# Mistra-UEA/Mistra

Measured on AMD Instinct MI355X. Metric: chemistry-timesteps/sec (tot mechanism), higher is better.
Workload: dtype f64; 1 GPU; tot mechanism, 100000 synthetic cells per GPU (100000 total), INTEGRATE_t(0,10 s), Ros3 rtol 1e-3; perturbed captured BTZ96 cloud states; cells_per_gpu=100000, failed_cells=0, parallelism=cells sharded over 1 GPU(s), no data-path collective

## Files before the change

### __graft_entry__.py

```python
import os
import subprocess
import sys

REPO = os.path.dirname(os.path.abspath(__file__))
if REPO not in sys.path:
    sys.path.insert(0, REPO)


def build():
    from mistra_amd.build import build_lib
    lib = build_lib()
    assert os.path.exists(lib)
    subprocess.run(["make", "-s", "-C", os.path.join(REPO, "oracle")], check=True)
    subprocess.run(["make", "-s", "-C", os.path.join(REPO, "tests", "emu")], check=True)
    if os.path.isdir("/root/reference/src") and not os.path.exists(os.path.join(REPO, "oracle", "_ref", "libmistra_ref.so")):
        subprocess.run([os.path.join(REPO, "oracle", "build_ref.sh"), "lib"], check=True)
    if os.path.isdir("/root/reference/src") and not os.path.exists(os.path.join(REPO, "oracle", "_ref", "mistra_two_pass")):
        subprocess.run([os.path.join(REPO, "oracle", "build_ref.sh"), "model"], check=True)
        subprocess.run([os.path.join(REPO, "oracle", "build_two_pass.sh")], check=True)
    if os.path.isdir("/root/reference/src") and not os.path.exists(os.path.join(REPO, "oracle", "_ref", "mistra_drive")):
        subprocess.run([os.path.join(REPO, "oracle", "build_drive.sh")], check=True)
    gpu_model = os.path.join(REPO, "oracle", "_ref", "mistra_gpu")
    if os.path.isdir("/root/reference/src"):
        srcs = [os.path.join(REPO, "shim", f) for f in os.listdir(os.path.join(REPO, "shim")) if f.endswith(".f90")]
        srcs += [os.path.join(REPO, "oracle", f) for f in ("column_driver.f90", "two_pass_patch.py", "build_gpu_model.sh")]
        if not os.path.exists(gpu_model) or any(os.path.getmtime(f) > os.path.getmtime(gpu_model) for f in srcs):
            if os.path.getmtime(os.path.join(REPO, "oracle", "column_driver.f90")) > os.path.getmtime(os.path.join(REPO, "oracle", "_ref", "obj", "column_driver.o")):
                subprocess.run([os.path.join(REPO, "oracle", "build_ref.sh"), "model"], check=True)
            subprocess.run([os.path.join(REPO, "oracle", "build_gpu_model.sh")], check=True)
    import mistra_amd
    from mistra_amd import chem
    chem.lib()


def smoke():
    import numpy as np
    import torch
    from mistra_amd import chem
    from oracle.oracle import Oracle
    assert torch.cuda.is_available(), "smoke() needs a GPU"
    chem.init(0)
    for mech, n in (("tot", 8), ("gas", 4)):
        z = np.load(os.path.join(REPO, "tests", "golden", "integrate_%s.npz" % mech))
        var, fix, rconst = z["var_in"][:n], z["fix"][:n], z["rconst"][:n]
        dev = torch.device("cuda", 0)
        res = chem.integrate(mech, torch.tensor(var, device=dev), torch.tensor(fix, device=dev), torch.tensor(rconst, device=dev))
        torch.cuda.synchronize()
        got = res.var.cpu().numpy()
        want, ierr, st = Oracle(mech).integrate_batch(var, fix, rconst)
        assert np.all(res.ierr.cpu().numpy() == 1) and np.all(ierr == 1)
        floor = 1e-12 * np.abs(want).max(axis=1, keepdims=True)
        rel = np.abs(got - want) / (np.abs(want) + floor)
        assert rel.max() < 1e-6, "smoke parity failed for %s: %g" % (mech, rel.max())
        assert np.array_equal(res.stats.cpu().numpy()[:, 2], st[:, 2]), "step counts differ from the oracle"
        print("smoke %s: %d cells, max rel diff vs oracle %.3e, steps %s" % (mech, n, rel.max(), st[:, 2].tolist()))


if __name__ == "__main__":
    build()
    if "--smoke" in sys.argv:
        smoke()
```

### mistra_amd/csrc/capi.cpp

```cpp
#include "../../include/mistra_chem.h"

#include <dlfcn.h>
#include <hip/hip_runtime.h>

#include <algorithm>
#include <cstdio>
#include <cstdlib>
#include <cstring>
#include <mutex>
#include <string>
#include <thread>
#include <vector>

#include "kernel_args.hpp"
#include "mech_tables.hpp"
#include "pack.hpp"
#include "rates.hpp"
#include "ros3_kernel.hpp"
#include "schedule.hpp"

using namespace mistra;

namespace {

// ... 93 lines not shown
bool mistra::PackTable::load(const std::string& path, std::string* err) {
  FILE* f = std::fopen(path.c_str(), "rb");
  if (!f) { if (err) *err = "cannot open " + path; return false; }
  int32_t h[16];
  bool ok = std::fread(h, sizeof h, 1, f) == 1 && h[0] == 0x4B41504B && h[1] == 1;
  for (int i = 2; ok && i < 16; i++) ok = h[i] >= 0 && h[i] <= (1 << 20);
  ok = ok && h[2] > 0 && h[3] >= 0 && h[4] > 0 && h[5] > 0 && h[6] >= 1 && h[6] <= 8 && h[7] <= 1 && h[11] <= kBudSlots;
  auto rd = [&](std::vector<int32_t>& v, size_t n) { v.resize(n); return n == 0 || std::fread(v.data(), 4, n, f) == n; };
  if (ok) {
    nvar = h[2]; nfix = h[3]; j2 = h[4]; j6 = h[5]; nkc = h[6]; preclamp = h[7];
    ok = rd(pack, (size_t)h[8] * 4) && rd(fix, (size_t)h[9] * 3) && rd(unpack, (size_t)h[10] * 4) && rd(slot_id, (size_t)h[11]) &&
         rd(slot_first, (size_t)h[11] + 1) && rd(terms, (size_t)h[12] * 3) && rd(term_words, (size_t)h[13]) && rd(acc, (size_t)h[14] * 2) &&
         rd(envc, (size_t)h[15] * 2);
  }
  std::fclose(f);
  if (ok) {
    const int nspec = nvar + nfix, nl = j2 * nkc, ni = j6 * nkc, nterms = (int)terms.size() / 3, nwords = (int)term_words.size();
    for (int i = 0; ok && i < n_pack(); i++) {
      const int32_t* e = &pack[(size_t)4 * i];
      ok = e[0] >= 0 && e[0] < nspec && (e[1] == 0 || e[1] == 1) && e[2] >= 0 && e[2] < (e[1] == 0 ? nl : ni) && (e[3] == 0 || e[3] == 1);
    }
    for (int i = 0; ok && i < n_fix(); i++) {
      const int32_t* e = &fix[(size_t)3 * i];
      ok = e[0] >= 0 && e[0] < nspec && e[1] >= 0 && e[1] <= 3 && e[2] >= 0 && e[2] < 4;
    }
    for (int i = 0; ok && i < n_unpack(); i++) {
      const int32_t* e = &unpack[(size_t)4 * i];
      ok = (e[0] == 0 || e[0] == 1) && e[1] >= 0 && e[1] < (e[0] == 0 ? nl : ni) && e[2] >= 0 && e[2] < nvar && (e[3] == 0 || e[3] == 1);
    }
    for (int i = 0; ok && i < n_slots(); i++)
      ok = slot_id[(size_t)i] >= 1 && slot_id[(size_t)i] <= kBudSlots && slot_first[(size_t)i] >= 0 && slot_first[(size_t)i] <= slot_first[(size_t)i + 1] &&
           slot_first[(size_t)i + 1] <= nterms;
    for (int q = 0; ok && q < nterms; q++) {
      const int w0 = terms[(size_t)3 * q + 2], w1 = q + 1 < nterms ? terms[(size_t)3 * (q + 1) + 2] : nwords;
      ok = terms[(size_t)3 * q + 1] >= 0 && w0 >= 0 && w0 <= w1 && w1 <= nwords;
    }
    for (int32_t w : term_words) ok = ok && w >= 0 && w < nvar;
    for (size_t a = 0; ok && a < acc.size() / 2; a++) ok = acc[2 * a] >= 1 && acc[2 * a] <= acc[2 * a + 1] && acc[2 * a + 1] <= kBudSlots;
    for (int i = 0; ok && i < n_envc(); i++) ok = envc[(size_t)2 * i] >= 0 && envc[(size_t)2 * i + 1] >= 0 && envc[(size_t)2 * i + 1] < nspec;
  }
  if (!ok && err) *err = path + ": not a hand-over table";
  return ok;
}

bool mistra::KmtTable::load(const std::string& path, std::string* err) {
  FILE* f = std::fopen(path.c_str(), "r");
  if (!f) { if (err) *err = "cannot open " + path; return false; }
  bool ok = std::fscanf(f, "%d %d %d %d", &nx, &nka, &nkt, &nkc) == 4 && nx > 0 && nx <= 64;
  if (ok) {
    lex.resize((size_t)nx);
    for (int i = 0; ok && i < nx; i++) ok = std::fscanf(f, "%d", &lex[(size_t)i]) == 1;
  }
  std::fclose(f);
  if (!ok && err) *err = path + ": not a species list of fast_k_mt";
  return ok;
}

bool mistra::LiqTable::load(const std::string& path, std::string* err) {
  FILE* f = std::fopen(path.c_str(), "rb");
  if (!f) { if (err) *err = "cannot open " + path; return false; }
  int32_t h[8];
  double d[3];
  bool ok = std::fread(h, sizeof h, 1, f) == 1 && h[0] == 0x5451494C && h[1] == 1 && h[2] > 0 && h[2] <= 4096 && h[3] >= 0 && h[3] <= h[2] &&
            h[4] >= 0 && h[4] <= h[2] && h[5] >= 1 && h[5] <= 8 && h[6] >= 0 && h[6] <= 1 << 20 && std::fread(d, sizeof d, 1, f) == 1;
  std::vector<int32_t> hj, hk, ej;
  std::vector<double> a0, b0;
  auto rdi = [&](std::vector<int32_t>& v, size_t n) { v.resize(n); return n == 0 || std::fread(v.data(), 4, n, f) == n; };
  auto rdd = [&](std::vector<double>& v, size_t n) { v.resize(n); return n == 0 || std::fread(v.data(), 8, n, f) == n; };
  if (ok) {
    nspec = h[2]; nh = h[3]; ne = h[4]; nkc_eq = h[5]; nfac = h[6];
    henry_tref = d[0]; henry_fct = d[1]; equil_tref = d[2];
    ok = rdi(hj, (size_t)nh) && rdi(hk, (size_t)nh) && rdd(a0, (size_t)nh) && rdd(b0, (size_t)nh) && rdi(ej, (size_t)ne) && rdi(foff, (size_t)ne + 1) &&
         rdi(boff, (size_t)ne + 1) && rdi(fkind, (size_t)nfac) && rdi(farg, (size_t)nfac) && rdd(fa, (size_t)nfac) && rdd(fb, (size_t)nfac);
  }
  std::fclose(f);
  if (ok) {
    h_kind.assign((size_t)nspec, -1); h_a0.assign((size_t)nspec, 0.0); h_b0.assign((size_t)nspec, 0.0); e_of.assign((size_t)nspec, -1);
    for (int i = 0; ok && i < nh; i++) {
      ok = hj[(size_t)i] >= 1 && hj[(size_t)i] <= nspec && (hk[(size_t)i] == 0 || hk[(size_t)i] == 1);
      if (ok) { const size_t j = (size_t)hj[(size_t)i] - 1; h_kind[j] = hk[(size_t)i]; h_a0[j] = a0[(size_t)i]; h_b0[j] = b0[(size_t)i]; }
    }
    for (int i = 0; ok && i < ne; i++) {
      ok = ej[(size_t)i] >= 1 && ej[(size_t)i] <= nspec && foff[(size_t)i] >= 0 && foff[(size_t)i] < boff[(size_t)i] && boff[(size_t)i] < foff[(size_t)i + 1] &&
           foff[(size_t)i + 1] <= nfac;
      if (ok) e_of[(size_t)ej[(size_t)i] - 1] = i;
    }
    for (int i = 0; ok && i < nfac; i++) ok = fkind[(size_t)i] >= 0 && fkind[(size_t)i] <= 3 && (fkind[(size_t)i] != 3 || (farg[(size_t)i] >= 1 && farg[(size_t)i] <= 4096));
  }
  if (!ok && err) *err = path + ": not a table of Henry / equilibrium constants";
  return ok;
}

bool mistra::VmeanTable::load(const std::string& path, std::string* err) {
  FILE* f = std::fopen(path.c_str(), "rb");
  if (!f) { if (err) *err = "cannot open " + path; return false; }
  int32_t h[8];
  bool ok = std::fread(h, sizeof h, 1, f) == 1 && h[0] == 0x544E4D56 && h[1] == 1 && h[2] > 0 && h[2] <= 4096 && h[3] >= 0 && h[3] <= h[2] &&
            std::fread(&coef, sizeof coef, 1, f) == 1 && coef > 0.0;
  std::vector<int32_t> j;
  std::vector<double> m;
  if (ok) {
    nspec = h[2];
    j.resize((size_t)h[3]); m.resize((size_t)h[3]);
    ok = (h[3] == 0 || std::fread(j.data(), 4, j.size(), f) == j.size()) && (h[3] == 0 || std::fread(m.data(), 8, m.size(), f) == m.size());
  }
  std::fclose(f);
  if (ok) {
    mass.assign((size_t)nspec, 0.0);
    for (size_t i = 0; ok && i < j.size(); i++) {
      ok = j[i] >= 1 && j[i] <= nspec && m[i] > 0.0;
      if (ok) mass[(size_t)j[i] - 1] = m[i];
    }
  }
  if (!ok && err) *err = path + ": not a table of molar masses of v_mean";
  return ok;
}

namespace {

struct VmBufs {
  DevBuf<uint32_t> wave_base, recs;
  DevBuf<uint16_t> blk_n;
  int nrounds = 0;
  hipError_t upload(const VmProgram& P) {
    nrounds = P.nbarriers;
    hipError_t e;
    if ((e = wave_base.upload(P.wave_base)) != hipSuccess) return e;
    if ((e = blk_n.upload(P.blk_n)) != hipSuccess) return e;
    return recs.upload(P.recs);
  }
  VmDev dev() const { return VmDev{wave_base.p, blk_n.p, recs.p, nrounds}; }
  void release() { wave_base.release(); recs.release(); blk_n.release(); }
};

struct GsBufs {
  DevBuf<uint32_t> wave_base, recs;
  DevBuf<uint16_t> rows;
  hipError_t upload(const GsumProgram& P) {
    hipError_t e;
    if ((e = wave_base.upload(P.wave_base)) != hipSuccess) return e;
    if ((e = rows.upload(P.rows)) != hipSuccess) return e;
    return recs.upload(P.recs);
  }
  GsDev dev() const { return GsDev{wave_base.p, rows.p, recs.p}; }
  void release() { wave_base.release(); recs.release(); rows.release(); }
};


struct KernelBufs {
  int n_temps = 0, lu_scale_slots = 0;
  DevBuf<double> consts;
  DevBuf<uint64_t> fun_fac, jac_fac;
  DevBuf<uint16_t> jvs_pos, zero_pos, diag_pos, schur_cells;
  GsBufs vdot, jvs;
  VmBufs lu, solve_head_fwd, solve_head_bwd;
  DevBuf<uint32_t> tail_fwd, tail_bwd, tail_fwd_addr[2], tail_bwd_addr[2], lu_scale, dense_rows;
  int upload(const MechTables& t, const KernelSchedule& K) {
    n_temps = K.n_temps;
    lu_scale_slots = K.lu_scale.nslots;
    HIP_TRY(consts.upload(t.consts));
    HIP_TRY(fun_fac.upload(K.fun_fac));
    HIP_TRY(jac_fac.upload(K.jac_fac));
    HIP_TRY(jvs_pos.upload(K.jvs_pos));
    HIP_TRY(zero_pos.upload(K.zero_pos));
    HIP_TRY(diag_pos.upload(K.diag_pos));
    HIP_TRY(vdot.upload(K.vdot));
    HIP_TRY(jvs.upload(K.jvs));
    HIP_TRY(lu.upload(K.lu));
    HIP_TRY(solve_head_fwd.upload(K.solve_head_fwd));
    HIP_TRY(solve_head_bwd.upload(K.solve_head_bwd));
    HIP_TRY(tail_fwd.upload(K.tail.fwd));
    HIP_TRY(tail_bwd.upload(K.tail.bwd));
    for (int r = 0; r < 2; r++) {
      HIP_TRY(tail_fwd_addr[r].upload(K.tail.fwd_addr[r]));
      HIP_TRY(tail_bwd_addr[r].upload(K.tail.bwd_addr[r]));
    }
    HIP_TRY(lu_scale.upload(K.lu_scale.recs));
    HIP_TRY(dense_rows.upload(K.dense.row_info));
    HIP_TRY(schur_cells.upload(K.dense.schur_cells));
    return 0;
  }
  void release() {
    consts.release(); fun_fac.release(); jac_fac.release(); jvs_pos.release(); zero_pos.release(); diag_pos.release(); schur_cells.release();
    vdot.release(); jvs.release(); lu.release(); solve_head_fwd.release(); solve_head_bwd.release();
    tail_fwd.release(); tail_bwd.release(); lu_scale.release(); dense_rows.release();
    for (int r = 0; r < 2; r++) { tail_fwd_addr[r].release(); tail_bwd_addr[r].release(); }
  }
};

struct RatesBufs {
  bool ready = false;
  int nreact = 0, nenv = 0;
  DevBuf<double> consts;
  DevBuf<int32_t> offs, words, fslot;
  int upload(const RatesTable& T) {
    HIP_TRY(consts.upload(T.consts));
    HIP_TRY(offs.upload(T.offs));
    HIP_TRY(words.upload(T.words));
    HIP_TRY(fslot.upload(T.fslot));
    nreact = T.nreact; nenv = T.nenv;
    ready = true;
    return 0;
  }
  RatesDev dev() const { return RatesDev{consts.p, offs.p, words.p, fslot.p, nreact, nenv}; }
  void release() { consts.release(); offs.release(); words.release(); fslot.release(); ready = false; }
};

struct PackBufs {
  bool ready = false, maps_ready = false;
  PackTable tab;
  DevBuf<int32_t> pack, fix, unpack, slot_id, slot_first, terms, words, acc, envc, a_ptr, a_fac;
  DevBuf<int32_t> gas_m2k, gas_k2m, rad_m2k, rad_k2m;
  int j1 = 0, j5 = 0;
  int upload(const MechTables& t) {
    HIP_TRY(pack.upload(tab.pack)); HIP_TRY(fix.upload(tab.fix)); HIP_TRY(unpack.upload(tab.unpack));
    HIP_TRY(slot_id.upload(tab.slot_id)); HIP_TRY(slot_first.upload(tab.slot_first)); HIP_TRY(terms.upload(tab.terms));
    HIP_TRY(words.upload(tab.term_words)); HIP_TRY(acc.upload(tab.acc)); HIP_TRY(envc.upload(tab.envc));
    HIP_TRY(a_ptr.upload(t.a_ptr)); HIP_TRY(a_fac.upload(t.a_fac));
    ready = true;
    return 0;
  }
  int set_maps(int n1, const int32_t* g_m2k, const int32_t* g_k2m, int n5, const int32_t* r_m2k, const int32_t* r_k2m) {
    HIP_TRY(gas_m2k.upload(std::vector<int32_t>(g_m2k, g_m2k + 2 * (size_t)n1)));
    HIP_TRY(gas_k2m.upload(std::vector<int32_t>(g_k2m, g_k2m + (size_t)n1)));
    HIP_TRY(rad_m2k.upload(std::vector<int32_t>(r_m2k, r_m2k + 2 * (size_t)n5)));
    HIP_TRY(rad_k2m.upload(std::vector<int32_t>(r_k2m, r_k2m + (size_t)n5)));
    j1 = n1; j5 = n5;
    maps_ready = true;
    return 0;
  }
  PackDev dev(int nreact, const double* consts) const {
    const PackTable& T = tab;
    return PackDev{pack.p, fix.p, unpack.p, slot_id.p, slot_first.p, terms.p, words.p, acc.p, envc.p,
                   T.n_pack(), T.n_fix(), T.n_unpack(), T.n_slots(), (int)T.terms.size() / 3, (int)T.term_words.size(), (int)T.acc.size() / 2, T.n_envc(),
                   T.nvar, T.nfix, nreact, T.j2, T.j6, T.nkc, T.preclamp, gas_m2k.p, gas_k2m.p, rad_m2k.p, rad_k2m.p, j1, j5, a_ptr.p, a_fac.p, consts};
  }
  void release() {
    pack.release(); fix.release(); unpack.release(); slot_id.release(); slot_first.release(); terms.release(); words.release(); acc.release();
    envc.release(); a_ptr.release(); a_fac.release(); gas_m2k.release(); gas_k2m.release(); rad_m2k.release(); rad_k2m.release();
    ready = maps_ready = false;
  }
};

struct KmtBufs {
  bool ready = false;
  KmtTable tab;
  DevBuf<int32_t> lex;
  int upload() {
    HIP_TRY(lex.upload(tab.lex));
    ready = true;
    return 0;
  }
  KmtDev dev(int nspec, int ka, int ifeed, int nkc_l) const { return KmtDev{lex.p, {0}, tab.nx, tab.nka, tab.nkt, tab.nkc, nspec, ka, ifeed, nkc_l}; }
  void release() { lex.release(); ready = false; }
};

struct LiqBufs {
  bool ready = false;
  LiqTable tab;
  DevBuf<int32_t> h_kind, e_of, foff, boff, fkind, farg;
  DevBuf<double> h_a0, h_b0, fa, fb;
  int upload() {
    HIP_TRY(h_kind.upload(tab.h_kind)); HIP_TRY(e_of.upload(tab.e_of)); HIP_TRY(foff.upload(tab.foff)); HIP_TRY(boff.upload(tab.boff));
    HIP_TRY(fkind.upload(tab.fkind)); HIP_TRY(farg.upload(tab.farg)); HIP_TRY(h_a0.upload(tab.h_a0)); HIP_TRY(h_b0.upload(tab.h_b0));
    HIP_TRY(fa.upload(tab.fa)); HIP_TRY(fb.upload(tab.fb));
    ready = true;
    return 0;
  }
  LiqDev dev() const {
    return LiqDev{h_kind.p, e_of.p, foff.p, boff.p, fkind.p, farg.p, h_a0.p, h_b0.p, fa.p, fb.p, tab.nspec, tab.nkc_eq, tab.henry_tref, tab.henry_fct, tab.equil_tref};
  }
  void release() {
    h_kind.release(); e_of.release(); foff.release(); boff.release(); fkind.release(); farg.release(); h_a0.release(); h_b0.release();
    fa.release(); fb.release(); ready = false;
  }
};

struct StcBufs {
  bool ready = false;
  StcoeffTable tab;
  DevBuf<double> consts[4];
  DevBuf<int32_t> offs[4], words[4];
  int upload() {
    for (int i = 0; i < 4; i++) {
      HIP_TRY(consts[i].upload(tab.v[i].consts)); HIP_TRY(offs[i].upload(tab.v[i].offs)); HIP_TRY(words[i].upload(tab.v[i].words));
    }
    ready = true;
    return 0;
  }
  RatesDev dev(int v) const { return RatesDev{consts[v].p, offs[v].p, words[v].p, nullptr, tab.v[v].nreact, tab.v[v].nenv}; }
  void release() {
    for (int i = 0; i < 4; i++) { consts[i].release(); offs[i].release(); words[i].release(); }
    ready = false;
  }
};

struct VmeanBufs {
  bool ready = false;
  VmeanTable tab;
  DevBuf<double> mass;
  int upload() {
    HIP_TRY(mass.upload(tab.mass));
    ready = true;
    return 0;
  }
  void release() { mass.release(); ready = false; }
};

enum : unsigned { kNeedRates = 1, kNeedPackTable = 2, kNeedMaps = 4, kNeedPack = kNeedPackTable | kNeedMaps, kNeedKmt = 8, kNeedLiq = 16, kNeedStc = 32, kNeedVmean = 64 };


struct Staging {
  char *dev = nullptr, *host = nullptr;
  size_t cap = 0;
  hipStream_t st = nullptr;
  hipError_t ensure(size_t bytes) {
    if (!st)
      if (hipError_t e = hipStreamCreateWithFlags(&st, hipStreamNonBlocking)) return e;
    if (bytes <= cap) return hipSuccess;
    free_blocks();
    const size_t want = bytes + bytes / 2;
    if (hipError_t e = hipMalloc(reinterpret_cast<void**>(&dev), want)) return e;
    if (hipError_t e = hipHostMalloc(reinterpret_cast<void**>(&host), want, hipHostMallocDefault)) return e;
    cap = want;
    return hipSuccess;
  }
  template <class T = double>
  T* d(size_t off) const { return reinterpret_cast<T*>(dev + off); }
  template <class T = double>
  T* h(size_t off) const { return reinterpret_cast<T*>(host + off); }
  void free_blocks() {
    if (dev) (void)hipFree(dev);
    if (host) (void)hipHostFree(host);
    dev = host = nullptr; cap = 0;
  }
  void release() {
    free_blocks();
    if (st) (void)hipStreamDestroy(st);
    st = nullptr;
  }
};

struct Layout {
  size_t end = 0;
  size_t take(size_t bytes) {
    const size_t at = end;
    end += (bytes + 255) & ~(size_t)255;
    return at;
  }
};

struct DriveLayout {
  size_t nl = 0, j1 = 0, j5 = 0, nsl = 0, nsi = 0, nv = 0, nf = 0, nr = 0, ne = 0;
  size_t s1 = 0, s3 = 0, sl1 = 0, si = 0, bg = 0, bgs = 0, io_end = 0, scal = 0, env = 0, in_end = 0;
  size_t th = 0, hl = 0, ierr = 0, stats = 0, cp = 0, out_end = 0, var = 0, fix = 0, rct = 0, end = 0;
};

struct MechState {
  bool ready = false;
  int nt = 0;
  MechTables tab;
  std::string text;
  KernelBufs k;
  RatesBufs rates;
  PackBufs pack;
  KmtBufs kmt;
  LiqBufs liq;
  StcBufs stc;
  VmeanBufs vmean;
  DevBuf<double> d_rct;
  DevBuf<double> s_var, s_fix, s_rct, s_th, s_env;
  DevBuf<int32_t> s_ierr, s_stats, s_sing;
  size_t sing_start = 0, sing_count = 0;
  bool sing_one = false;
  int32_t one_sing[8] = {0, 0, 0, 0, 0, 0, 0, 0};
  Staging drive;
  Staging one;
  struct PendingDrive {
    bool active = false;
    DriveLayout lay;
    std::vector<int32_t> layer, level;
    double *s1 = nullptr, *s3 = nullptr, *sl1 = nullptr, *sion1 = nullptr, *bg = nullptr, *bgs = nullptr, *t_h = nullptr, *c_packed = nullptr;
    int32_t *ierr = nullptr, *stats = nullptr;
    int nrxn = 0;
  } pend;
  void release() {
    k.release(); rates.release(); pack.release(); kmt.release(); liq.release(); stc.release(); vmean.release();
    d_rct.release();
    s_var.release(); s_fix.release(); s_rct.release(); s_th.release(); s_env.release(); s_ierr.release(); s_stats.release(); s_sing.release();
    sing_count = 0; sing_one = false;
    drive.release(); one.release();
    pend = PendingDrive{};
    ready = false;
  }
};

struct DeviceState {
  int id = -1;
  MechState mech[3];
  bool lds_configured[3] = {false, false, false};
  void release() {
    if (id >= 0) (void)hipSetDevice(id);
    for (auto& m : mech) m.release();
    for (bool& c : lds_configured) c = false;
    id = -1;
  }
};

std::mutex g_mu;
bool g_inited = false;
int g_max_steps = 100000;
std::vector<DeviceState> g_devs;

Staging g_liq;
struct PinnedRanges {
  std::vector<std::pair<const char*, size_t>> r;
  bool contains(const void* p, size_t n) const {
    const char* c = static_cast<const char*>(p);
    for (const auto& x : r)
      if (c >= x.first && c + n <= x.first + x.second) return true;
    return false;
  }
  void release() {
    for (const auto& x : r) (void)hipHostUnregister(const_cast<char*>(x.first));
    r.clear();
  }
} g_pinned;

void release_all() {
  if (!g_devs.empty() && g_devs[0].id >= 0) (void)hipSetDevice(g_devs[0].id);
  g_pinned.release();
  g_liq.release();
  for (auto& d : g_devs) d.release();
  g_devs.clear();
  g_inited = false;
}

std::string mech_dir() {
  if (const char* e = std::getenv("MISTRA_MECH_DIR")) return e;
  Dl_info info;
  if (dladdr(reinterpret_cast<const void*>(&mistra_chem_init), &info) && info.dli_fname) {
    std::string p = info.dli_fname;
    size_t k = p.rfind('/');
    std::string dir = k == std::string::npos ? "." : p.substr(0, k);
    return dir + "/../mech";
  }
  return "mech";
}

int default_nt(int mech) { return mech == MISTRA_MECH_GAS ? kGasNT : mech == MISTRA_MECH_AER ? kAerNT : kTotNT; }

template <class MT>
bool traits_match(const MechTables& t, int n_jnz, int tail_regs, bool scale_pass, const DenseTail& dense) {
  return dense.nd == MT::DENSE_ND && dense.kb == MT::DENSE_KB && tail_regs == MT::TAIL_REGS && scale_pass == MT::SCALE_PASS && t.nvar == MT::NVAR && t.nfix == MT::NFIX && t.nreact == MT::NREACT && t.nnz == MT::NNZ && t.nb == MT::NB &&
         t.nconst == MT::NCONST && n_jnz == MT::NJNZ;
}

int setup_mech(DeviceState& D, int mech) {
  MechState& S = D.mech[mech];
  const std::string name = kMechName[mech], base = mech_dir() + "/" + name;
  std::string err;
  if (!S.tab.load(base + ".mech", &err)) return fail(err);
  S.nt = default_nt(mech);
  const bool nt_ok = (mech == MISTRA_MECH_GAS && S.nt == kGasNT) || (mech == MISTRA_MECH_AER && S.nt == kAerNT) ||
                     (mech == MISTRA_MECH_TOT && S.nt == kTotNT);
  if (!nt_ok) return fail(std::string("no kernel instantiated for workgroup size ") + std::to_string(S.nt) + " of " + kMechName[mech]);
  const uint32_t ab_base = 8u * (uint32_t)(mech == MISTRA_MECH_GAS   ? LdsLayout<GasTraits, kGasNT>::AB
                                           : mech == MISTRA_MECH_AER ? LdsLayout<AerTraits, kAerNT>::AB
                                                                     : LdsLayout<TotTraits, kTotNT>::AB);
  KernelSchedule K;
  try {
    const int max_temps = mech == MISTRA_MECH_GAS ? GasTraits::MAX_TEMPS : mech == MISTRA_MECH_AER ? AerTraits::MAX_TEMPS : TotTraits::MAX_TEMPS;
    const DenseConfig dc = dense_config(S.tab);
    const uint32_t jb_base = 8u * (uint32_t)(mech == MISTRA_MECH_GAS   ? LdsLayout<GasTraits, kGasNT>::JB
                                             : mech == MISTRA_MECH_AER ? LdsLayout<AerTraits, kAerNT>::JB
                                                                       : LdsLayout<TotTraits, kTotNT>::JB);
    K = build_kernel_schedule(S.tab, S.nt, ab_base, max_temps, dc.nd, dc.kb, jb_base);
  } catch (const std::exception& ex) {
    return fail(std::string("schedule compiler: ") + ex.what());
  }
  bool ok = mech == MISTRA_MECH_GAS   ? traits_match<GasTraits>(S.tab, K.n_jnz, K.tail.regs, K.lu_scale.nslots > 0, K.dense)
            : mech == MISTRA_MECH_AER ? traits_match<AerTraits>(S.tab, K.n_jnz, K.tail.regs, K.lu_scale.nslots > 0, K.dense)
                                      : traits_match<TotTraits>(S.tab, K.n_jnz, K.tail.regs, K.lu_scale.nslots > 0, K.dense);
  if (!ok) return fail(name + ": mechanism table does not match the compiled kernel sizes");
  S.text = name + ": " + describe(K);
  if (int rc = S.k.upload(S.tab, K)) return rc;
  const int nspec = S.tab.nvar + S.tab.nfix;
  RatesTable R;
  if (R.load(base + ".rates", &err)) {
    if (R.nreact != S.tab.nreact) return fail(name + ".rates does not belong to this mechanism");
    if (int rc = S.rates.upload(R)) return rc;
  }
  if (S.pack.tab.load(base + ".pack", &err)) {
    const PackTable& T = S.pack.tab;
    if (T.nvar != S.tab.nvar || T.nfix != S.tab.nfix) return fail(name + ".pack does not belong to this mechanism");
    for (size_t q = 0; q < T.terms.size() / 3; q++)
      if (T.terms[3 * q + 1] >= S.tab.nreact) return fail(name + ".pack: a budget term names a reaction the mechanism does not have");
    for (int i = 0; i < T.n_envc(); i++)
      if (S.rates.ready && T.envc[(size_t)2 * i] >= S.rates.nenv) return fail(name + ".pack: a concentration slot lies outside the rate evaluator's input");
    if (int rc = S.pack.upload(S.tab)) return rc;
  }
  if (S.kmt.tab.load(base + ".kmt", &err)) {
    for (int32_t i : S.kmt.tab.lex)
      if (i < 1 || i > nspec) return fail(name + ".kmt does not belong to this mechanism");
    if (int rc = S.kmt.upload()) return rc;
  }
  if (S.liq.tab.load(base + ".liq", &err)) {
    if (S.liq.tab.nspec != nspec) return fail(name + ".liq does not belong to this mechanism");
    if (int rc = S.liq.upload()) return rc;
  }
  if (S.stc.tab.load(base + ".stcoeff", &err)) {
    if (S.stc.tab.v[0].nreact != nspec) return fail(name + ".stcoeff does not belong to this mechanism");
    if (int rc = S.stc.upload()) return rc;
  }
  if (S.vmean.tab.load(base + ".vmean", &err)) {
    if (S.vmean.tab.nspec != nspec) return fail(name + ".vmean does not belong to this mechanism");
    if (int rc = S.vmean.upload()) return rc;
  }
  S.ready = true;
  return 0;
}

int launch(DeviceState& D, int mech, const KernelArgs& a, hipStream_t stream) {
  hipError_t e = hipErrorInvalidValue;
  if (mech == MISTRA_MECH_GAS) e = launch_ros3<GasTraits, kGasNT>(a, stream, &D.lds_configured[mech]);
  else if (mech == MISTRA_MECH_AER) e = launch_ros3<AerTraits, kAerNT>(a, stream, &D.lds_configured[mech]);
  else e = launch_ros3<TotTraits, kTotNT>(a, stream, &D.lds_configured[mech]);
  if (e != hipSuccess) return fail(std::string("kernel launch: ") + hipGetErrorString(e));
  return 0;
}

KernelArgs make_args(const MechState& S, int ncell, const double* var_in, const double* fix, const double* rconst, double tin,
                     double tout, double* var_out, int32_t* ierr, int32_t* stats, double* th) {
  const KernelBufs& k = S.k;
  KernelArgs a;
  a.var_in = var_in; a.fix = fix; a.rconst = rconst; a.var_out = var_out; a.ierr = ierr; a.stats = stats;
  a.texit_hexit = th; a.h_last = nullptr; a.hstart = nullptr; a.prof = nullptr; a.dump = nullptr; a.sing_rows = nullptr; a.n_temps = k.n_temps; a.max_steps = g_max_steps; a.tin = tin; a.tout = tout; a.ncell = ncell;
  a.consts = k.consts.p; a.fun_fac = k.fun_fac.p; a.jac_fac = k.jac_fac.p; a.jvs_pos = k.jvs_pos.p;
  a.zero_pos = k.zero_pos.p; a.diag_pos = k.diag_pos.p;
  a.vdot = k.vdot.dev(); a.jvs = k.jvs.dev(); a.lu = k.lu.dev();
#ifdef MISTRA_DIAG_ENV
  if (const char* cut = std::getenv("MISTRA_DIAG_LU_ROUNDS"))
    a.lu.nrounds = std::max(1, std::min(a.lu.nrounds, std::atoi(cut)));
#endif
  a.solve_head_fwd = k.solve_head_fwd.dev(); a.solve_head_bwd = k.solve_head_bwd.dev();
  a.tail = TailDev{k.tail_fwd.p, k.tail_bwd.p, {k.tail_fwd_addr[0].p, k.tail_fwd_addr[1].p}, {k.tail_bwd_addr[0].p, k.tail_bwd_addr[1].p}};
  a.lu_scale = ScaleDev{k.lu_scale.p, k.lu_scale_slots, k.lu_scale_slots + VM_LOOKAHEAD_ROWS};
  a.dense = DenseDev{k.dense_rows.p, k.schur_cells.p};
  return a;
}

PackDev pack_dev(const MechState& S) { return S.pack.dev(S.tab.nreact, S.k.consts.p); }

int check_call(int mech, int ncell) {
  if (mech < 0 || mech > 2) return fail("unknown mechanism id");
  if (ncell < 0) return fail("negative cell count");
  if (!g_inited || g_devs.empty() || !g_devs[0].mech[mech].ready) return fail("mistra_chem_init has not been called (or failed)");
  return 0;
}

int require(const MechState& S, int mech, unsigned need) {
  const std::string m = kMechName[mech];
  if ((need & kNeedPackTable) && !S.pack.ready) return fail("no hand-over table for the " + m + " mechanism");
  if ((need & kNeedMaps) && !S.pack.maps_ready) return fail("mistra_chem_set_species_maps has not been called for the " + m + " mechanism");
  if ((need & kNeedRates) && !S.rates.ready) return fail("no device rate table for the " + m + " mechanism");
  if ((need & kNeedKmt) && !S.kmt.ready) return fail("the " + m + " mechanism has no mass-transfer routine (fast_k_mt_a: aer, fast_k_mt_t: tot)");
  if ((need & kNeedLiq) && !S.liq.ready)
    return fail("the " + m + " mechanism has no liquid-phase routines (henry_a / equil_co_a: aer, henry_t / equil_co_t: tot)");
  if ((need & kNeedStc) && !S.stc.ready) return fail("the " + m + " mechanism has no st_coeff routine (st_coeff_a: aer, st_coeff_t: tot)");
  if ((need & kNeedVmean) && !S.vmean.ready) return fail("the " + m + " mechanism has no v_mean routine (v_mean_a: aer, v_mean_t: tot)");
  return 0;
}

struct Slot {
  DeviceState* D = nullptr;
  MechState* S = nullptr;
};

int on_device(int mech, int ncell, const void* p, const char* what, unsigned need, Slot* t) {
  if (int rc = check_call(mech, ncell)) return rc;
  hipPointerAttribute_t attr;
  if (hipPointerGetAttributes(&attr, p) != hipSuccess) return fail(std::string(what) + " is not a device pointer");
  DeviceState* D = nullptr;
  for (auto& d : g_devs)
    if (d.id == attr.device) { D = &d; break; }
  if (!D) return fail("the buffers live on device " + std::to_string(attr.device) + ", which mistra_chem_init(_devices) did not set up");
  if (int rc = require(D->mech[mech], mech, need)) return rc;
  HIP_TRY(hipSetDevice(D->id));
  *t = Slot{D, &D->mech[mech]};
  return 0;
}

int on_primary(int mech, unsigned need, bool mutates, Slot* t) {
  DeviceState& D = g_devs[0];
  MechState& S = D.mech[mech];
  if (mutates && S.pend.active)
    return fail(std::string("a column step of the ") + kMechName[mech] + " mechanism is open (mistra_chem_drive_begin): fetch it with mistra_chem_drive_end first");
  if (int rc = require(S, mech, need)) return rc;
  HIP_TRY(hipSetDevice(D.id));
  *t = Slot{&D, &S};
  return 0;
}

int init_locked(int n, const int* ids) {
  int count = 0;
  hipError_t e = hipGetDeviceCount(&count);
  if (e != hipSuccess || count <= 0) return fail("no HIP device available (this library has no CPU path)");
  if (n <= 0 || n > 64) return fail("device count out of range");
  std::vector<int> want((size_t)n);
  for (int i = 0; i < n; i++) {
    want[(size_t)i] = ids ? ids[i] : i;
    if (want[(size_t)i] < 0 || want[(size_t)i] >= count) return fail("device index out of range");
  }
  bool same = g_inited && g_devs.size() == want.size();
  for (size_t i = 0; same && i < want.size(); i++) same = g_devs[i].id == want[i];
  if (same) {
    HIP_TRY(hipSetDevice(g_devs[0].id));
    return 0;
  }
  release_all();
  g_devs.resize(want.size());
  for (size_t i = 0; i < want.size(); i++) {
    HIP_TRY(hipSetDevice(want[i]));
    g_devs[i].id = want[i];
    for (int mech = 0; mech < 3; mech++)
      if (int rc = setup_mech(g_devs[i], mech)) return rc;
  }
  HIP_TRY(hipSetDevice(g_devs[0].id));
  g_inited = true;
  return 0;
}

int integrate_host_on(DeviceState& D, int mech, int ncell, const double* var_in, const double* fix, const double* rconst, double tin,
                      double tout, double* var_out, int32_t* ierr, int32_t* stats, double* t_h, size_t batch_start = 0,
                      const double* env = nullptr) {
  HIP_TRY(hipSetDevice(D.id));
  MechState& S = D.mech[mech];
  const size_t nv = (size_t)kDims[mech].nvar, nf = (size_t)kDims[mech].nfix, nr = (size_t)kDims[mech].nreact, nc = (size_t)ncell;
  HIP_TRY(S.s_var.reserve(nc * nv));
  HIP_TRY(S.s_fix.reserve(nc * nf));
  HIP_TRY(S.s_rct.reserve(nc * nr));
  HIP_TRY(S.s_ierr.reserve(nc));
  HIP_TRY(S.s_stats.reserve(nc * 8));
  HIP_TRY(S.s_sing.reserve(nc * 8));
  if (t_h) HIP_TRY(S.s_th.reserve(nc * 3));
  HIP_TRY(hipMemcpy(S.s_var.p, var_in, nc * nv * sizeof(double), hipMemcpyHostToDevice));
  HIP_TRY(hipMemcpy(S.s_fix.p, fix, nc * nf * sizeof(double), hipMemcpyHostToDevice));
  if (env) {
    const size_t ne = (size_t)S.rates.nenv;
    HIP_TRY(S.s_env.reserve(nc * ne));
    HIP_TRY(hipMemcpy(S.s_env.p, env, nc * ne * sizeof(double), hipMemcpyHostToDevice));
    LAUNCH_TRY(launch_update_rconst(S.rates.dev(), S.s_env.p, S.s_rct.p, ncell, nullptr));
  } else {
    HIP_TRY(hipMemcpy(S.s_rct.p, rconst, nc * nr * sizeof(double), hipMemcpyHostToDevice));
  }
  KernelArgs a = make_args(S, ncell, S.s_var.p, S.s_fix.p, S.s_rct.p, tin, tout, S.s_var.p, S.s_ierr.p, S.s_stats.p, t_h ? S.s_th.p : nullptr);
  if (t_h) a.h_last = S.s_th.p + 2 * nc;
  a.sing_rows = S.s_sing.p;
  S.sing_start = batch_start; S.sing_count = nc; S.sing_one = false;
  DevBuf<unsigned long long> prof;
#ifdef MISTRA_DIAG_ENV
  const bool profile = std::getenv("MISTRA_CHEM_PROFILE") != nullptr;
#else
  const bool profile = false;
#endif
  if (profile) {
    HIP_TRY(prof.reserve(nc * kProfSlots));
    a.prof = prof.p;
  }
  if (int rc = launch(D, mech, a, nullptr)) return rc;
  HIP_TRY(hipDeviceSynchronize());
  if (profile) {
    std::vector<unsigned long long> h(nc * kProfSlots);
    HIP_TRY(hipMemcpy(h.data(), prof.p, nc * kProfSlots * sizeof(unsigned long long), hipMemcpyDeviceToHost));
    double sum[kProfSlots] = {0};
    for (size_t c = 0; c < nc; c++)
      for (int k = 0; k < kProfSlots; k++) sum[k] += (double)h[c * kProfSlots + k];
    const char* names[kProfSlots] = {"fun", "jac", "prepare", "lu", "solve(rest)", "norm", "other", "total", "solve_head_fwd", "solve_tail", "solve_head_bwd", "lu_scale", "lu_dense", "jac_products", "jac_sums", "fun_products"};
    std::fprintf(stderr, "[mistra_chem profile] %s, %zu cells, mean shader-clock ticks per cell:", kMechName[mech], nc);
    for (int k = 0; k < kProfSlots; k++) std::fprintf(stderr, " %s=%.0f (%.1f%%)", names[k], sum[k] / nc, 100.0 * sum[k] / sum[7]);
    std::fprintf(stderr, "\n");
    prof.release();
  }
  HIP_TRY(hipMemcpy(var_out, S.s_var.p, nc * nv * sizeof(double), hipMemcpyDeviceToHost));
  if (ierr) HIP_TRY(hipMemcpy(ierr, S.s_ierr.p, nc * sizeof(int32_t), hipMemcpyDeviceToHost));
  if (stats) HIP_TRY(hipMemcpy(stats, S.s_stats.p, nc * 8 * sizeof(int32_t), hipMemcpyDeviceToHost));
  if (t_h) {
    std::vector<double> h(nc * 3);
    HIP_TRY(hipMemcpy(h.data(), S.s_th.p, nc * 3 * sizeof(double), hipMemcpyDeviceToHost));
    for (size_t c = 0; c < nc; c++) { t_h[3 * c] = h[2 * c]; t_h[3 * c + 1] = h[2 * c + 1]; t_h[3 * c + 2] = h[2 * nc + c]; }
  }
  return 0;
}
// ... 871 lines not shown
```

### mistra_amd/csrc/kernel_args.hpp

```cpp
#pragma once
#include <cstdint>

namespace mistra {

constexpr int kProfSlots = 16;
constexpr int kVmSweepUpdPerRec = 3;

struct VmDev {
  const uint32_t* wave_base;
  const uint16_t* blk_n;
  const uint32_t* recs;
  int nrounds;
};

struct GsDev {
  const uint32_t* wave_base;
  const uint16_t* rows;
  const uint32_t* recs;
};

struct ScaleDev {
  const uint32_t* recs;
  int nslots;
  int wave_slots;
};

struct TailDev {
  const uint32_t* fwd;
  const uint32_t* bwd;
  const uint32_t* fwd_addr[2];
  const uint32_t* bwd_addr[2];
};

struct DenseDev {
  const uint32_t* row_info;
  const uint16_t* schur_cells;
};

struct KernelArgs {
  const double* var_in;
  const double* fix;
  const double* rconst;
  double* var_out;
  int32_t* ierr;
  int32_t* stats;
  double* texit_hexit;
  const double* hstart;
  double* h_last;
  int32_t* sing_rows;
  double* dump;
  unsigned long long* prof;
  double tin, tout;
  int32_t ncell;
  int32_t n_temps;
  int32_t max_steps;
  const double* consts;
  const uint64_t* fun_fac;
  const uint64_t* jac_fac;
  const uint16_t* jvs_pos;
  const uint16_t* zero_pos;
  const uint16_t* diag_pos;
  GsDev vdot, jvs;
  VmDev lu, solve_head_fwd, solve_head_bwd;
  ScaleDev lu_scale;
  TailDev tail;
  DenseDev dense;
};

}
```

### mistra_amd/csrc/ros3_kernel.hip

```cpp
#include <hip/hip_runtime.h>

#include <cstdint>
#include <type_traits>

#include "kernel_args.hpp"
#include "ros3_kernel.hpp"

namespace mistra {

namespace {

constexpr uint16_t kPosDiag = 0x8000, kPosNone = 0xFFFF;
constexpr int kRingSlots = 8;

typedef uint32_t u32x4 __attribute__((ext_vector_type(4)));
typedef float f32x4 __attribute__((ext_vector_type(4)));

template <class T>
using gptr = const T __attribute__((address_space(1)))*;
template <class T>
using gptr_mut = T __attribute__((address_space(1)))*;
template <class T>
__device__ __forceinline__ gptr<T> G_(const T* p) { return (gptr<T>)p; }
template <class T>
__device__ __forceinline__ gptr_mut<T> GM_(T* p) { return (gptr_mut<T>)p; }

typedef __attribute__((address_space(3))) double lds_f64;
__device__ __forceinline__ uint32_t lds_addr(const void* p) {
  return (uint32_t)(uintptr_t)(__attribute__((address_space(3))) const void*)p;
}
__device__ __forceinline__ double lds_ld(uint32_t addr) { return *(const lds_f64*)(uintptr_t)addr; }
__device__ __forceinline__ void lds_st(uint32_t addr, double v) { *(lds_f64*)(uintptr_t)addr = v; }

__device__ __forceinline__ void lds_barrier() {
  __builtin_amdgcn_fence(__ATOMIC_RELEASE, "workgroup", "local");
  __builtin_amdgcn_s_barrier();
  __builtin_amdgcn_fence(__ATOMIC_ACQUIRE, "workgroup", "local");
}

constexpr double kRosA1 = 1.0;
constexpr double kRosC1 = -0.10156171083877702091975600115545e+01;
constexpr double kRosC2 = 0.40759956452537699824805835358067e+01;
constexpr double kRosC3 = 0.92076794298330791242156818474003e+01;
constexpr double kRosM1 = 0.1e+01;
constexpr double kRosM2 = 0.61697947043828245592553615689730e+01;
constexpr double kRosM3 = -0.42772256543218573326238373806514e+00;
constexpr double kRosE1 = 0.5e+00;
constexpr double kRosE2 = -0.29079558716805469821718236208017e+01;
constexpr double kRosE3 = 0.22354069897811569627360909276199e+00;
constexpr double kRosGamma1 = 0.43586652150845899941601945119356e+00;
[[maybe_unused]] constexpr double kRosGamma2 = 0.24291996454816804366592249683314e+00;
[[maybe_unused]] constexpr double kRosGamma3 = 0.21851380027664058511513169485832e+01;
constexpr double kRosElo = 3.0;

__device__ __attribute__((noinline)) double err_root(double err) { return pow(err, 1.0 / kRosElo); }

__device__ __forceinline__ double wave_uniform(double v) {
  const uint64_t u = __builtin_bit_cast(uint64_t, v);
  const uint32_t lo = (uint32_t)__builtin_amdgcn_readfirstlane((int)(uint32_t)u), hi = (uint32_t)__builtin_amdgcn_readfirstlane((int)(uint32_t)(u >> 32));
  return __builtin_bit_cast(double, (uint64_t)lo | ((uint64_t)hi << 32));
}

__device__ __forceinline__ double scalar_const(double v) {
  const uint64_t u = __builtin_bit_cast(uint64_t, v);
  uint32_t lo = (uint32_t)u, hi = (uint32_t)(u >> 32);
  asm volatile("" : "+s"(lo), "+s"(hi));
  return __builtin_bit_cast(double, (uint64_t)lo | ((uint64_t)hi << 32));
}

template <int CTRL>
__device__ __forceinline__ double dpp_partner(double v) {
  const uint64_t u = __builtin_bit_cast(uint64_t, v);
  const int lo = __builtin_amdgcn_update_dpp(0, (int)(uint32_t)u, CTRL, 0xf, 0xf, false);
  const int hi = __builtin_amdgcn_update_dpp(0, (int)(uint32_t)(u >> 32), CTRL, 0xf, 0xf, false);
  return __builtin_bit_cast(double, (uint64_t)(uint32_t)lo | ((uint64_t)(uint32_t)hi << 32));
}
__device__ __forceinline__ double wave_sum(double v) {
  v += dpp_partner<0xB1>(v);
  v += dpp_partner<0x4E>(v);
  v += dpp_partner<0x141>(v);
  v += dpp_partner<0x140>(v);
  {
    const uint64_t u = __builtin_bit_cast(uint64_t, v);
    const auto l = __builtin_amdgcn_permlane16_swap((uint32_t)u, (uint32_t)u, false, false);
    const auto h = __builtin_amdgcn_permlane16_swap((uint32_t)(u >> 32), (uint32_t)(u >> 32), false, false);
    v = __builtin_bit_cast(double, (uint64_t)l[0] | ((uint64_t)h[0] << 32)) + __builtin_bit_cast(double, (uint64_t)l[1] | ((uint64_t)h[1] << 32));
  }
  {
    const uint64_t u = __builtin_bit_cast(uint64_t, v);
    const auto l = __builtin_amdgcn_permlane32_swap((uint32_t)u, (uint32_t)u, false, false);
    const auto h = __builtin_amdgcn_permlane32_swap((uint32_t)(u >> 32), (uint32_t)(u >> 32), false, false);
    v = __builtin_bit_cast(double, (uint64_t)l[0] | ((uint64_t)h[0] << 32)) + __builtin_bit_cast(double, (uint64_t)l[1] | ((uint64_t)h[1] << 32));
  }
  return v;
}

__device__ __forceinline__ double fmin_f(double a, double b) { return (a < b || b != b) ? a : b; }
__device__ __forceinline__ double fmax_f(double a, double b) { return (a > b || b != b) ? a : b; }

template <bool LOW, int K, int BYTE_OFFSET = 0>
__device__ __forceinline__ void vm_ring_load(gptr<u32x4> p) {
#define MISTRA_RING_LOAD(R0, R1, R2, R3)                                                                              \
  asm volatile("global_load_dwordx4 v[" #R0 ":" #R3 "], %0, off offset:%1" : : "v"(p), "n"(BYTE_OFFSET)             \
               : "memory", "v" #R0, "v" #R1, "v" #R2, "v" #R3)
  if constexpr (LOW) {
    if constexpr (K == 0) MISTRA_RING_LOAD(64, 65, 66, 67);
    else if constexpr (K == 1) MISTRA_RING_LOAD(68, 69, 70, 71);
    else if constexpr (K == 2) MISTRA_RING_LOAD(80, 81, 82, 83);
    else if constexpr (K == 3) MISTRA_RING_LOAD(84, 85, 86, 87);
    else if constexpr (K == 4) MISTRA_RING_LOAD(96, 97, 98, 99);
    else if constexpr (K == 5) MISTRA_RING_LOAD(100, 101, 102, 103);
    else if constexpr (K == 6) MISTRA_RING_LOAD(112, 113, 114, 115);
    else MISTRA_RING_LOAD(116, 117, 118, 119);
  } else {
    if constexpr (K == 0) MISTRA_RING_LOAD(192, 193, 194, 195);
    else if constexpr (K == 1) MISTRA_RING_LOAD(196, 197, 198, 199);
    else if constexpr (K == 2) MISTRA_RING_LOAD(208, 209, 210, 211);
    else if constexpr (K == 3) MISTRA_RING_LOAD(212, 213, 214, 215);
    else if constexpr (K == 4) MISTRA_RING_LOAD(224, 225, 226, 227);
    else if constexpr (K == 5) MISTRA_RING_LOAD(228, 229, 230, 231);
    else if constexpr (K == 6) MISTRA_RING_LOAD(240, 241, 242, 243);
    else MISTRA_RING_LOAD(244, 245, 246, 247);
  }
#undef MISTRA_RING_LOAD
}

struct RingBase { uint64_t b0, b1; };
__device__ __forceinline__ RingBase ring_base(const void* p) {
  const uint64_t u = (uint64_t)(uintptr_t)p;
  uint32_t lo, hi;
  asm volatile("v_readfirstlane_b32 %0, %2\n\tv_readfirstlane_b32 %1, %3\n\ts_nop 4" : "=s"(lo), "=s"(hi) : "v"((uint32_t)u), "v"((uint32_t)(u >> 32)));
  const uint64_t b = (uint64_t)lo | ((uint64_t)hi << 32);
  return RingBase{b, b + 4096};
}
__device__ __forceinline__ void ring_advance(RingBase& r, uint32_t bytes) { r.b0 += bytes; r.b1 += bytes; }
template <bool LOW, int K, int ROW>
__device__ __forceinline__ void vm_ring_load_s(const RingBase& r, uint32_t voff) {
  static_assert(ROW >= 0 && ROW <= 7, "row within the two 4-KiB windows");
#define MISTRA_RING_LOAD_S(R0, R1, R2, R3)                                                                                    \
  asm volatile("global_load_dwordx4 v[" #R0 ":" #R3 "], %0, %1 offset:%2" : : "v"(voff), "s"(ROW < 4 ? r.b0 : r.b1), "n"((ROW % 4) * 1024) \
               : "memory", "v" #R0, "v" #R1, "v" #R2, "v" #R3)
  if constexpr (LOW) {
    if constexpr (K == 0) MISTRA_RING_LOAD_S(64, 65, 66, 67);
    else if constexpr (K == 1) MISTRA_RING_LOAD_S(68, 69, 70, 71);
    else if constexpr (K == 2) MISTRA_RING_LOAD_S(80, 81, 82, 83);
    else if constexpr (K == 3) MISTRA_RING_LOAD_S(84, 85, 86, 87);
    else if constexpr (K == 4) MISTRA_RING_LOAD_S(96, 97, 98, 99);
    else if constexpr (K == 5) MISTRA_RING_LOAD_S(100, 101, 102, 103);
    else if constexpr (K == 6) MISTRA_RING_LOAD_S(112, 113, 114, 115);
    else MISTRA_RING_LOAD_S(116, 117, 118, 119);
  } else {
    if constexpr (K == 0) MISTRA_RING_LOAD_S(192, 193, 194, 195);
    else if constexpr (K == 1) MISTRA_RING_LOAD_S(196, 197, 198, 199);
    else if constexpr (K == 2) MISTRA_RING_LOAD_S(208, 209, 210, 211);
    else if constexpr (K == 3) MISTRA_RING_LOAD_S(212, 213, 214, 215);
    else if constexpr (K == 4) MISTRA_RING_LOAD_S(224, 225, 226, 227);
    else if constexpr (K == 5) MISTRA_RING_LOAD_S(228, 229, 230, 231);
    else if constexpr (K == 6) MISTRA_RING_LOAD_S(240, 241, 242, 243);
    else MISTRA_RING_LOAD_S(244, 245, 246, 247);
  }
#undef MISTRA_RING_LOAD_S
}

template <bool LOW, int K, int IMM>
__device__ __forceinline__ void vm_ring_load_at(uint64_t sbase, uint32_t voff) {
  static_assert(IMM >= 0 && IMM < 4096, "13-bit signed immediate offset");
#define MISTRA_RING_LOAD_AT(R0, R1, R2, R3)                                                                                   \
  asm volatile("global_load_dwordx4 v[" #R0 ":" #R3 "], %0, %1 offset:%2" : : "v"(voff), "s"(sbase), "n"(IMM)                \
               : "memory", "v" #R0, "v" #R1, "v" #R2, "v" #R3)
// ... 396 lines not shown
    } else {
      base = tb[0] + (uint64_t)(TS::NB + G - TS::NG) * 4096u;
    }
    vm_ring_load_at<LOW, K0, 0>(base, voff); vm_ring_load_at<LOW, K0 + 1, 1024>(base, voff);
    vm_ring_load_at<LOW, K0 + 2, 2048>(base, voff); vm_ring_load_at<LOW, K0 + 3, 3072>(base, voff);
  };
  asm volatile("s_waitcnt vmcnt(0)" : : : "memory");
  load(std::integral_constant<int, 0>());
  load(std::integral_constant<int, 1>());
  double c[16];
  {
    double g[16];
    tail_gather<LOW, 0>(g);
    load(std::integral_constant<int, 2>());
#pragma unroll
    for (int j = 0; j < 16; j++) c[j] = g[TS::bw(0) ? 15 - j : j];
  }
#define MISTRA_TAIL_STEP(S)                                                                                               \
  if constexpr ((S) < TS::NS) {                                                                                          \
    if constexpr ((S) == TS::NF) {                                                                                       \
      _Pragma("unroll") for (int r = 0; r < R; r++) x[r] = x[r] * rd[r];                                                 \
    }                                                                                                                    \
    tail_block<TS, (S), LOW>(x, c, load);                                                                                \
  }
  MISTRA_TAIL_STEP(0) MISTRA_TAIL_STEP(1) MISTRA_TAIL_STEP(2) MISTRA_TAIL_STEP(3) MISTRA_TAIL_STEP(4) MISTRA_TAIL_STEP(5) MISTRA_TAIL_STEP(6) MISTRA_TAIL_STEP(7)
  MISTRA_TAIL_STEP(8) MISTRA_TAIL_STEP(9) MISTRA_TAIL_STEP(10) MISTRA_TAIL_STEP(11) MISTRA_TAIL_STEP(12) MISTRA_TAIL_STEP(13) MISTRA_TAIL_STEP(14) MISTRA_TAIL_STEP(15)
#undef MISTRA_TAIL_STEP
  asm volatile("s_waitcnt vmcnt(0)" : : : "memory");
#pragma unroll
  for (int r = 0; r < R; r++) lds_st(xb + 8 * (r * 64 + lane), x[r]);
}

__device__ __forceinline__ double readlane_f64(double v, int l) {
  const uint64_t u = __builtin_bit_cast(uint64_t, v);
  const uint32_t lo = (uint32_t)__builtin_amdgcn_readlane((int)(uint32_t)u, l);
  const uint32_t hi = (uint32_t)__builtin_amdgcn_readlane((int)(uint32_t)(u >> 32), l);
  return __builtin_bit_cast(double, (uint64_t)lo | ((uint64_t)hi << 32));
}

template <int R, int FWD_FROM, bool LOW>
__device__ __attribute__((noinline)) void tail_solve_columns(const TailDev T, uint32_t xb, uint32_t rb, int lane) {
  constexpr int FWD_END = R;
  constexpr bool FORWARD = FWD_FROM < FWD_END;
  constexpr uint32_t mb = 0;
  double x[R], rd[R];
  const uint32_t voff = 16u * (uint32_t)lane;
  static_assert(R == 1 || R == 2, "one or two 64-row registers");
  uint32_t three = 3;
  asm volatile("" : "+v"(three));
#pragma unroll
  for (int r = 0; r < R; r++) x[r] = lds_ld(xb + 8 * (r * 64 + lane));
#define MISTRA_TAIL_OPERANDS(BUF, K, PENDING)                                           \
  {                                                                                     \
    uint32_t alo[4], ahi[4];                                                            \
    vm_ring_take_cells<LOW, K, PENDING, true, R == 2>(alo, ahi, three);                 \
    _Pragma("unroll") for (int c = 0; c < 4; c++) {                                     \
      BUF[c][0] = lds_ld(mb + alo[c]);                                                  \
      if constexpr (R == 2) BUF[c][1] = lds_ld(mb + ahi[c]);                            \
    }                                                                                   \
  }
#define MISTRA_TAIL_PIN _Pragma("unroll") for (int r = 0; r < R; r++) asm volatile("" : "+v"(x[r]));
  double opa[4][R], opb[4][R];
  if constexpr (FORWARD) {
    RingBase tp = ring_base(T.fwd + FWD_FROM * 16 * 64 * 4);
    asm volatile("s_waitcnt vmcnt(0)" : : : "memory");
    vm_ring_load_s<LOW, 0, 0>(tp, voff); vm_ring_load_s<LOW, 1, 1>(tp, voff); vm_ring_load_s<LOW, 2, 2>(tp, voff); vm_ring_load_s<LOW, 3, 3>(tp, voff);
    vm_ring_load_s<LOW, 4, 4>(tp, voff); vm_ring_load_s<LOW, 5, 5>(tp, voff); vm_ring_load_s<LOW, 6, 6>(tp, voff); vm_ring_load_s<LOW, 7, 7>(tp, voff);
    ring_advance(tp, kRingSlots * 1024);
    MISTRA_TAIL_OPERANDS(opa, 0, 7)
    vm_ring_load_s<LOW, 0, 0>(tp, voff);
#pragma unroll
    for (int rq = FWD_FROM; rq < FWD_END; rq++) {
      for (int gb = 0; gb < 16; gb += kRingSlots) {
#define MISTRA_TAIL_FWD(K, CUR, NXT)                                                    \
        {                                                                               \
          MISTRA_TAIL_OPERANDS(NXT, (K + 1) % kRingSlots, 7)                                 \
          if constexpr (K + 1 == kRingSlots) ring_advance(tp, kRingSlots * 1024);            \
          vm_ring_load_s<LOW, (K + 1) % kRingSlots, (K + 1) % kRingSlots>(tp, voff);         \
          _Pragma("unroll") for (int c = 0; c < 4; c++) {                               \
            const double xq = readlane_f64(x[rq], 4 * (gb + K) + c);                    \
            _Pragma("unroll") for (int r = rq; r < R; r++) x[r] = __builtin_fma(-CUR[c][r], xq, x[r]); \
          }                                                                             \
          MISTRA_TAIL_PIN                                                               \
        }
        MISTRA_TAIL_FWD(0, opa, opb) MISTRA_TAIL_FWD(1, opb, opa) MISTRA_TAIL_FWD(2, opa, opb) MISTRA_TAIL_FWD(3, opb, opa)
        MISTRA_TAIL_FWD(4, opa, opb) MISTRA_TAIL_FWD(5, opb, opa) MISTRA_TAIL_FWD(6, opa, opb) MISTRA_TAIL_FWD(7, opb, opa)
#undef MISTRA_TAIL_FWD
      }
    }
  }
  {
    RingBase tp = ring_base(T.bwd);
    asm volatile("s_waitcnt vmcnt(0)" : : : "memory");
    vm_ring_load_s<LOW, 0, 0>(tp, voff); vm_ring_load_s<LOW, 1, 1>(tp, voff); vm_ring_load_s<LOW, 2, 2>(tp, voff); vm_ring_load_s<LOW, 3, 3>(tp, voff);
    vm_ring_load_s<LOW, 4, 4>(tp, voff); vm_ring_load_s<LOW, 5, 5>(tp, voff); vm_ring_load_s<LOW, 6, 6>(tp, voff); vm_ring_load_s<LOW, 7, 7>(tp, voff);
    ring_advance(tp, kRingSlots * 1024);
#pragma unroll
    for (int r = 0; r < R; r++) rd[r] = lds_ld(rb + 8 * (r * 64 + lane));
#pragma unroll
    for (int r = 0; r < R; r++) x[r] = x[r] * rd[r];
    MISTRA_TAIL_OPERANDS(opa, 0, 7)
    vm_ring_load_s<LOW, 0, 0>(tp, voff);
#pragma unroll
    for (int rq = R - 1; rq >= 0; rq--) {
      for (int gb = 0; gb < 16; gb += kRingSlots) {
#define MISTRA_TAIL_BWD(K, CUR, NXT)                                                    \
        {                                                                               \
          MISTRA_TAIL_OPERANDS(NXT, (K + 1) % kRingSlots, 7)                                 \
          if constexpr (K + 1 == kRingSlots) ring_advance(tp, kRingSlots * 1024);            \
          vm_ring_load_s<LOW, (K + 1) % kRingSlots, (K + 1) % kRingSlots>(tp, voff);         \
          _Pragma("unroll") for (int c = 0; c < 4; c++) {                               \
            const double xq = readlane_f64(x[rq], 63 - (4 * (gb + K) + c));             \
            _Pragma("unroll") for (int r = 0; r <= rq; r++) x[r] = __builtin_fma(-CUR[c][r], xq, x[r]); \
          }                                                                             \
          MISTRA_TAIL_PIN                                                               \
        }
        MISTRA_TAIL_BWD(0, opa, opb) MISTRA_TAIL_BWD(1, opb, opa) MISTRA_TAIL_BWD(2, opa, opb) MISTRA_TAIL_BWD(3, opb, opa)
        MISTRA_TAIL_BWD(4, opa, opb) MISTRA_TAIL_BWD(5, opb, opa) MISTRA_TAIL_BWD(6, opa, opb) MISTRA_TAIL_BWD(7, opb, opa)
#undef MISTRA_TAIL_BWD
      }
    }
  }
#undef MISTRA_TAIL_OPERANDS
#undef MISTRA_TAIL_PIN
  asm volatile("s_waitcnt vmcnt(0)" : : : "memory");
#pragma unroll
  for (int r = 0; r < R; r++) lds_st(xb + 8 * (r * 64 + lane), x[r]);
}

#include "gsum_exec_asm.inc"
template <int NT, bool LOW>
__device__ __attribute__((noinline)) void gsum_run(const GsDev P, uint32_t row0, int rows, int lane, uint32_t out_addr, uint32_t out_stride) {
  int n = __builtin_amdgcn_readfirstlane(rows);
  const uint64_t recs = reinterpret_cast<uint64_t>(P.recs) + (uint64_t)(uint32_t)__builtin_amdgcn_readfirstlane((int)row0) * 2048u;
  const uint64_t b0 = (uint64_t)(uint32_t)__builtin_amdgcn_readfirstlane((int)(uint32_t)recs) |
                      ((uint64_t)(uint32_t)__builtin_amdgcn_readfirstlane((int)(uint32_t)(recs >> 32)) << 32);
  const uint64_t b1 = b0 + 4096u;
  uint32_t voff = (uint32_t)lane * 32u;
  double acc = -0.0;
  const double mzero = -0.0;
  double xA0, xA1, xA2, xA3, xB0, xB1, xB2, xB3, cA0, cA1, cA2, cA3, cB0, cB1, cB2, cB3;
  uint32_t ad, flA, flB;
#define MISTRA_GSUM_OPERANDS                                                                                                                   \
  [acc] "+&v"(acc), [ad] "=&v"(ad), [xA0] "=&v"(xA0), [xA1] "=&v"(xA1), [xA2] "=&v"(xA2), [xA3] "=&v"(xA3), [xB0] "=&v"(xB0), [xB1] "=&v"(xB1),    \
      [xB2] "=&v"(xB2), [xB3] "=&v"(xB3), [cA0] "=&v"(cA0), [cA1] "=&v"(cA1), [cA2] "=&v"(cA2), [cA3] "=&v"(cA3), [cB0] "=&v"(cB0),               \
      [cB1] "=&v"(cB1), [cB2] "=&v"(cB2), [cB3] "=&v"(cB3), [flA] "=&s"(flA), [flB] "=&s"(flB), [n] "+s"(n), [voff] "+&v"(voff),               \
      [out] "+&v"(out_addr)                                                                                                                    \
      : [b0] "s"(b0), [b1] "s"(b1), [stride] "v"(out_stride), [mzero] "v"(mzero)
  if constexpr (LOW) asm volatile(MISTRA_GSUM_ASM_LOW : MISTRA_GSUM_OPERANDS : "memory", "scc", MISTRA_GSUM_CLOBBER_LOW);
  else asm volatile(MISTRA_GSUM_ASM_HIGH : MISTRA_GSUM_OPERANDS : "memory", "scc", MISTRA_GSUM_CLOBBER_HIGH);
#undef MISTRA_GSUM_OPERANDS
}

template <int NT, bool LOW>
__device__ __attribute__((noinline)) void scale_run(const ScaleDev P, int wave, int lane) {
  const int n = __builtin_amdgcn_readfirstlane(P.nslots);
  gptr<u32x4> rp = G_(reinterpret_cast<const u32x4*>(P.recs)) + ((size_t)wave * (size_t)P.wave_slots * 64 + lane);
  asm volatile("s_waitcnt vmcnt(0)" : : : "memory");
  vm_ring_load<LOW, 0>(rp);       vm_ring_load<LOW, 1>(rp + 64);  vm_ring_load<LOW, 2>(rp + 128); vm_ring_load<LOW, 3>(rp + 192);
  vm_ring_load<LOW, 4>(rp + 256); vm_ring_load<LOW, 5>(rp + 320); vm_ring_load<LOW, 6>(rp + 384); vm_ring_load<LOW, 7>(rp + 448);
  rp += kRingSlots * 64;
  for (int i = 0; i < n; i += kRingSlots) {
#define MISTRA_SCALE_GROUP(K)                                                        \
    {                                                                                \
      const u32x4 a0 = vm_ring_take<LOW, K>();     vm_ring_load<LOW, K>(rp + K * 64);         \
      const u32x4 a1 = vm_ring_take<LOW, K + 1>(); vm_ring_load<LOW, K + 1>(rp + (K + 1) * 64); \
      const u32x4 a2 = vm_ring_take<LOW, K + 2>(); vm_ring_load<LOW, K + 2>(rp + (K + 2) * 64); \
      const u32x4 a3 = vm_ring_take<LOW, K + 3>(); vm_ring_load<LOW, K + 3>(rp + (K + 3) * 64); \
      const double v0 = lds_ld(a0.x), f0 = lds_ld(a0.y), v1 = lds_ld(a0.z), f1 = lds_ld(a0.w); \
      const double v2 = lds_ld(a1.x), f2 = lds_ld(a1.y), v3 = lds_ld(a1.z), f3 = lds_ld(a1.w); \
      const double v4 = lds_ld(a2.x), f4 = lds_ld(a2.y), v5 = lds_ld(a2.z), f5 = lds_ld(a2.w); \
      const double v6 = lds_ld(a3.x), f6 = lds_ld(a3.y), v7 = lds_ld(a3.z), f7 = lds_ld(a3.w); \
      lds_st(a0.x, v0 * f0); lds_st(a0.z, v1 * f1); lds_st(a1.x, v2 * f2); lds_st(a1.z, v3 * f3); \
      lds_st(a2.x, v4 * f4); lds_st(a2.z, v5 * f5); lds_st(a3.x, v6 * f6); lds_st(a3.z, v7 * f7); \
    }
    MISTRA_SCALE_GROUP(0) MISTRA_SCALE_GROUP(4)
#undef MISTRA_SCALE_GROUP
    rp += kRingSlots * 64;
  }
  asm volatile("s_waitcnt vmcnt(0)" : : : "memory");
}

#ifdef MISTRA_DIAG_STAMPS
__device__ unsigned long long g_dense_stamps[16];
#define MISTRA_STAMP(var) const unsigned long long var = clock64();
#define MISTRA_STAMP_ADD(slot, expr) if (threadIdx.x == 0) atomicAdd(&g_dense_stamps[slot], (unsigned long long)(expr));
#else
#define MISTRA_STAMP(var)
#define MISTRA_STAMP_ADD(slot, expr)
#endif
typedef double f64x4 __attribute__((ext_vector_type(4)));
typedef uint32_t u32x2 __attribute__((ext_vector_type(2)));
typedef __attribute__((address_space(3))) f64x4 lds_f64x4;
__device__ __forceinline__ f64x4 lds_ld4(uint32_t addr) { return *(const lds_f64x4*)(uintptr_t)addr; }
__device__ __forceinline__ void lds_st4(uint32_t addr, f64x4 v) { *(lds_f64x4*)(uintptr_t)addr = v; }

__device__ __forceinline__ uint32_t dense_slot(const u32x4 info, const uint32_t c, const uint32_t zero) {
  const uint64_t absent = (uint64_t)info.y | ((uint64_t)info.z << 32);
  const uint32_t idx = info.x + c - (uint32_t)__builtin_popcountll(absent & ((1ull << c) - 1ull));
  return ((absent >> c) & 1ull) ? zero : 8u * idx;
}
typedef __attribute__((address_space(3))) u32x4 lds_u32x4;
__device__ __forceinline__ u32x4 lds_ldu4(uint32_t addr) { return *(const lds_u32x4*)(uintptr_t)addr; }

__device__ __forceinline__ bool dense_is_storer(const int wave) { return wave == 1 || wave == 2 || wave == 3 || wave == 5; }
template <class MT, int NT>
__device__ __forceinline__ void dense_store_panel(const int P, const int wave, const int lane) {
  constexpr uint32_t NNZ = MT::NNZ, NVAR = MT::NVAR, H = NVAR - 64, ZERO = 8u * (NNZ + NVAR);
  constexpr uint32_t PB = 8u * (uint32_t)LdsLayout<MT, NT>::PANEL, BC = PB + 8192u, INFO = 8u * (uint32_t)LdsLayout<MT, NT>::DINFO;
  const uint32_t PL = PB + (uint32_t)(P & 1) * 4096u, PU = PL + 2048u;
  const int J0P = 4 * P, khalf = (wave == 3 || wave == 5) ? 2 : 0;
  const f64x4 rcp = lds_ld4(BC + 1024u + 32u * (uint32_t)(P & 1));
  if (wave & 1) {
    if (wave != 5) {
      const f64x4 a = lds_ld4(PL + 32u * lane);
      const u32x4 mine = lds_ldu4(INFO + 16u * lane);
      const double a0 = khalf ? a[2] : a[0], a1 = khalf ? a[3] : a[1];
      const uint32_t at0 = dense_slot(mine, (uint32_t)(J0P + khalf), ZERO), at1 = dense_slot(mine, (uint32_t)(J0P + khalf + 1), ZERO);
      if (lane > J0P + khalf && at0 != ZERO) lds_st(at0, a0);
      if (lane > J0P + khalf + 1 && at1 != ZERO) lds_st(at1, a1);
      if (wave == 1 && lane >= J0P && lane < J0P + 4) {
        const int k = lane - J0P;
        lds_st(8u * (NNZ + NVAR + 4u + H + (uint32_t)lane), k == 0 ? rcp[0] : k == 1 ? rcp[1] : k == 2 ? rcp[2] : rcp[3]);
      }
      return;
    }
  }
  {
    const f64x4 b = lds_ld4(PU + 32u * lane);
    const double b0 = khalf ? b[2] : b[0], b1 = khalf ? b[3] : b[1], r0 = khalf ? rcp[2] : rcp[0], r1 = khalf ? rcp[3] : rcp[1];
    const uint32_t at0 = dense_slot(lds_ldu4(INFO + 16u * (uint32_t)(J0P + khalf)), (uint32_t)lane, ZERO);
    const uint32_t at1 = dense_slot(lds_ldu4(INFO + 16u * (uint32_t)(J0P + khalf + 1)), (uint32_t)lane, ZERO);
    if (lane >= J0P + khalf && at0 != ZERO) lds_st(at0, lane == J0P + khalf ? b0 : b0 * r0);
    if (lane >= J0P + khalf + 1 && at1 != ZERO) lds_st(at1, lane == J0P + khalf + 1 ? b1 : b1 * r1);
  }
}

template <class MT, int NT>
__device__ __forceinline__ void dense_panel(f64x4& T0, f64x4& T1, const int P, const int wave, const int lane
#ifdef MISTRA_DIAG_STAMPS
                                            , unsigned long long (&acc)[5]
#endif
) {
  const int K = P >> 2, S = P & 3, J0P = 4 * P, K2 = (J0P + 4) >> 4;
  constexpr uint32_t PB = 8u * (uint32_t)LdsLayout<MT, NT>::PANEL, BC = PB + 8192u;
  const uint32_t PL = PB + (uint32_t)(P & 1) * 4096u, PU = PL + 2048u;
  const int I = wave >> 1, J0 = 2 * (wave & 1);
  const uint32_t lrow = (uint32_t)(lane >> 4), lcol = (uint32_t)(lane & 15);
  MISTRA_STAMP(ta)
  if (I >= K && (wave & 1) == (K >> 1)) {
    const bool odd = K & 1;
    const double t0 = odd ? T1[0] : T0[0], t1 = odd ? T1[1] : T0[1], t2 = odd ? T1[2] : T0[2], t3 = odd ? T1[3] : T0[3];
    if ((int)(lcol >> 2) == S) {
      const uint32_t at = PL + 8u * ((16u * I + lrow) * 4u + (lcol & 3u));
      lds_st(at, t0); lds_st(at + 128u, t1); lds_st(at + 256u, t2); lds_st(at + 384u, t3);
    }
  }
  if (I == K) {
    if (J0 >= K) lds_st(PU + 8u * ((16u * J0 + lcol) * 4u + lrow), S == 0 ? T0[0] : S == 1 ? T0[1] : S == 2 ? T0[2] : T0[3]);
    if (J0 + 1 >= K) lds_st(PU + 8u * ((16u * (J0 + 1) + lcol) * 4u + lrow), S == 0 ? T1[0] : S == 1 ? T1[1] : S == 2 ? T1[2] : T1[3]);
  }
  lds_barrier();
  MISTRA_STAMP(tb)
  if (wave == 0) {
    f64x4 a = lds_ld4(PL + 32u * lane), b = lds_ld4(PU + 32u * lane);
    const f64x4 c0 = lds_ld4(PU + 32u * (uint32_t)J0P), c1 = lds_ld4(PU + 32u * (uint32_t)(J0P + 1));
    const f64x4 c2 = lds_ld4(PU + 32u * (uint32_t)(J0P + 2)), c3 = lds_ld4(PU + 32u * (uint32_t)(J0P + 3));
    f64x4 rcp;
    rcp[0] = 1.0 / c0[0];
    const double l10 = c0[1] * rcp[0], l20 = c0[2] * rcp[0], l30 = c0[3] * rcp[0];
    const double u01 = c1[0], u02 = c2[0], u03 = c3[0];
    const double d11 = __builtin_fma(-l10, u01, c1[1]), d12 = __builtin_fma(-l10, u02, c2[1]), d13 = __builtin_fma(-l10, u03, c3[1]);
    double d21 = __builtin_fma(-l20, u01, c1[2]), d22 = __builtin_fma(-l20, u02, c2[2]), d23 = __builtin_fma(-l20, u03, c3[2]);
    double d31 = __builtin_fma(-l30, u01, c1[3]), d32 = __builtin_fma(-l30, u02, c2[3]), d33 = __builtin_fma(-l30, u03, c3[3]);
    rcp[1] = 1.0 / d11;
    const double l21 = d21 * rcp[1], l31 = d31 * rcp[1];
    d22 = __builtin_fma(-l21, d12, d22); d23 = __builtin_fma(-l21, d13, d23);
    d32 = __builtin_fma(-l31, d12, d32); d33 = __builtin_fma(-l31, d13, d33);
    rcp[2] = 1.0 / d22;
    const double l32 = d32 * rcp[2];
    d33 = __builtin_fma(-l32, d23, d33);
    rcp[3] = 1.0 / d33;
    a[0] = a[0] * rcp[0];
    a[1] = __builtin_fma(-a[0], u01, a[1]); a[2] = __builtin_fma(-a[0], u02, a[2]); a[3] = __builtin_fma(-a[0], u03, a[3]);
    a[1] = a[1] * rcp[1];
    a[2] = __builtin_fma(-a[1], d12, a[2]); a[3] = __builtin_fma(-a[1], d13, a[3]);
    a[2] = a[2] * rcp[2];
    a[3] = __builtin_fma(-a[2], d23, a[3]);
    a[3] = a[3] * rcp[3];
    b[1] = __builtin_fma(-l10, b[0], b[1]); b[2] = __builtin_fma(-l20, b[0], b[2]); b[3] = __builtin_fma(-l30, b[0], b[3]);
    b[2] = __builtin_fma(-l21, b[1], b[2]); b[3] = __builtin_fma(-l31, b[1], b[3]);
    b[3] = __builtin_fma(-l32, b[2], b[3]);
    lds_st4(PL + 32u * lane, a);
    lds_st4(PU + 32u * lane, b);
    if (lane == 0) lds_st4(BC + 1024u + 32u * (uint32_t)(P & 1), rcp);
  } else if (dense_is_storer(wave) && P > 0) {
    dense_store_panel<MT, NT>(P - 1, wave, lane);
  }
  MISTRA_STAMP(tc)
  lds_barrier();
  MISTRA_STAMP(td)
  if (I >= K2) {
    const double aop = (int)(16u * I + lcol) >= J0P + 4 ? -lds_ld(PL + 8u * ((16u * I + lcol) * 4u + lrow)) : 0.0;
    if (J0 >= K2) {
      const double bop = (int)(16u * J0 + lcol) >= J0P + 4 ? lds_ld(PU + 8u * ((16u * J0 + lcol) * 4u + lrow)) : 0.0;
      T0 = __builtin_amdgcn_mfma_f64_16x16x4f64(aop, bop, T0, 0, 0, 0);
    }
    if (J0 + 1 >= K2) {
      const double bop = (int)(16u * (J0 + 1) + lcol) >= J0P + 4 ? lds_ld(PU + 8u * ((16u * (J0 + 1) + lcol) * 4u + lrow)) : 0.0;
      T1 = __builtin_amdgcn_mfma_f64_16x16x4f64(aop, bop, T1, 0, 0, 0);
    }
  }
  MISTRA_STAMP(te)
#ifdef MISTRA_DIAG_STAMPS
  acc[0] += tb - ta; acc[1] += tc - tb; acc[2] += td - tc; acc[3] += te - td; acc[4] += 1;
#endif
}

template <class MT, int NT>
__device__ __attribute__((noinline)) void dense_lu(int lane) {
  static_assert(NT == 512 && MT::DENSE_ND == 64, "eight waves, two 16x16 tiles each");
  constexpr int KB = MT::DENSE_KB;
  constexpr uint32_t NNZ = MT::NNZ, NVAR = MT::NVAR, H = NVAR - 64, JM = H - 4 * KB, ZERO = 8u * (NNZ + NVAR);
  constexpr uint32_t INFO = 8u * (uint32_t)LdsLayout<MT, NT>::DINFO, RDIAG = 8u * (NNZ + NVAR + 4u);
  const int wave = __builtin_amdgcn_readfirstlane((int)(threadIdx.x >> 6));
  const uint32_t I = (uint32_t)(wave >> 1), J0 = 2u * (uint32_t)(wave & 1), lrow = (uint32_t)(lane >> 4), lcol = (uint32_t)(lane & 15);
  MISTRA_STAMP(t0)
  f64x4 T0, T1;
#pragma unroll
  for (int r = 0; r < 4; r++) {
    const u32x4 info = lds_ldu4(INFO + 16u * (16u * I + lrow + 4u * r));
    T0[r] = lds_ld(dense_slot(info, 16u * J0 + lcol, ZERO));
    T1[r] = lds_ld(dense_slot(info, 16u * J0 + 16u + lcol, ZERO));
  }
  constexpr uint32_t SCH = 8u * (uint32_t)LdsLayout<MT, NT>::SCHUR;
  typedef __attribute__((address_space(3))) uint16_t lds_u16;
  const uint32_t wtab = SCH + 2u * ((uint32_t)I * KB * 64u + (uint32_t)lane);
  const uint32_t utab = SCH + 2u * (4u * KB * 64u + (uint32_t)(wave & 1) * KB * 128u + (uint32_t)lane);
  uint32_t wslot[KB];
  double wl[KB];
  static_assert(KB % 2 == 0, "two batches of Schur steps");
#pragma unroll
  for (int half = 0; half < 2; half++) {
    constexpr int HB = KB / 2;
    uint32_t us0[HB], us1[HB];
#pragma unroll
    for (int kk = 0; kk < HB; kk++) {
      const int k = half * HB + kk;
      wslot[k] = 8u * (uint32_t)*(const lds_u16*)(uintptr_t)(wtab + 128u * k);
      us0[kk] = 8u * (uint32_t)*(const lds_u16*)(uintptr_t)(utab + 256u * k);
      us1[kk] = 8u * (uint32_t)*(const lds_u16*)(uintptr_t)(utab + 256u * k + 128u);
    }
    __builtin_amdgcn_sched_barrier(0);
    double u0[HB], u1[HB];
#pragma unroll
    for (int kk = 0; kk < HB; kk++) {
      wl[half * HB + kk] = lds_ld(wslot[half * HB + kk]);
      u0[kk] = lds_ld(us0[kk]);
      u1[kk] = lds_ld(us1[kk]);
    }
    __builtin_amdgcn_sched_barrier(0);
#pragma unroll
    for (int kk = 0; kk < HB; kk++) {
      T0 = __builtin_amdgcn_mfma_f64_16x16x4f64(-wl[half * HB + kk], u0[kk], T0, 0, 0, 0);
      T1 = __builtin_amdgcn_mfma_f64_16x16x4f64(-wl[half * HB + kk], u1[kk], T1, 0, 0, 0);
    }
  }
  double rj[KB / 2];
#pragma unroll
  for (int k2 = 0; k2 < KB / 2; k2++) rj[k2] = lds_ld(RDIAG + 8u * (JM + 4u * (2u * k2 + (uint32_t)(wave & 1)) + lrow));
  MISTRA_STAMP(t1)
  lds_barrier();
  {
    static_assert(KB % 2 == 0, "the two waves of a block row take every other Schur step");
    if (wave & 1) {
#pragma unroll
      for (int k = 1; k < KB; k += 2)
        if (wslot[k] != ZERO) lds_st(wslot[k], wl[k] * rj[k / 2]);
    } else {
#pragma unroll
      for (int k = 0; k < KB; k += 2)
        if (wslot[k] != ZERO) lds_st(wslot[k], wl[k] * rj[k / 2]);
    }
  }
  MISTRA_STAMP(t2)
  MISTRA_STAMP_ADD(0, t1 - t0) MISTRA_STAMP_ADD(1, t2 - t1) MISTRA_STAMP_ADD(9, 1)
#ifndef MISTRA_DENSE_UNROLL
#define MISTRA_DENSE_UNROLL 8
#endif
#ifndef MISTRA_DIAG_DENSE_PANELS
#define MISTRA_DIAG_DENSE_PANELS 16
#endif
#ifdef MISTRA_DIAG_STAMPS
  unsigned long long acc[5] = {0, 0, 0, 0, 0};
  MISTRA_STAMP(tp0)
#pragma unroll 1
  for (int P = 0; P < MISTRA_DIAG_DENSE_PANELS; P++) dense_panel<MT, NT>(T0, T1, P, wave, lane, acc);
  MISTRA_STAMP(tp1)
  MISTRA_STAMP_ADD(2, acc[0]) MISTRA_STAMP_ADD(3, acc[1]) MISTRA_STAMP_ADD(4, acc[2]) MISTRA_STAMP_ADD(5, acc[3]) MISTRA_STAMP_ADD(8, acc[4]) MISTRA_STAMP_ADD(12, tp1 - tp0)
#else
#pragma unroll MISTRA_DENSE_UNROLL
  for (int P = 0; P < MISTRA_DIAG_DENSE_PANELS; P++) dense_panel<MT, NT>(T0, T1, P, wave, lane);
#endif
  if (dense_is_storer(wave)) dense_store_panel<MT, NT>(15, wave, lane);
#ifdef MISTRA_DIAG_STAMPS
  lds_barrier();
  MISTRA_STAMP(tz)
  MISTRA_STAMP_ADD(11, tz - t0)
#endif
}

}

template <class MT, int NT, int VARIANT>
__global__ __launch_bounds__(NT, MT::WAVES_PER_SIMD) void ros3_integrate_kernel(const KernelArgs a) {
  constexpr bool PROF = VARIANT == 1, DUMP = VARIANT == 2;
  constexpr int NVAR = MT::NVAR, NFIX = MT::NFIX, NREACT = MT::NREACT, NNZ = MT::NNZ, NCONST = MT::NCONST;
  constexpr int NW = NT / 64;
  constexpr int SPT = (NVAR + NT - 1) / NT, RPT = (NREACT + NT - 1) / NT;
  constexpr int JPT = (MT::NJNZ + NT - 1) / NT, ZPT = (NNZ - MT::NJNZ + NT - 1) / NT;
  using L = LdsLayout<MT, NT>;

  extern __shared__ __attribute__((aligned(16))) double lds[];
  double* const M = lds + L::M;
  double* const XS = M + NNZ;
  double* const X = lds + L::X;
  double* const AB = lds + L::AB;
  double* const JBp = lds + L::JB;
  double* const red = lds + L::RED;
  int* const flags = reinterpret_cast<int*>(lds + L::FLAGS);

  const int t = threadIdx.x, lane = t & 63, wave = t >> 6;
  const int cell = blockIdx.x;
  if (cell >= a.ncell) return;
  if (lds_addr(lds) != 0u) {
    if (t == 0) GM_(a.ierr)[cell] = -99;
    return;
  }

  struct { uint32_t lu_row0, fwd_row0, bwd_row0, vdot_row0, jvs_row0; int vdot_rows, jvs_rows; } hdr;
  {
    const auto u = [](uint32_t v) { return (uint32_t)__builtin_amdgcn_readfirstlane((int)v); };
    hdr.lu_row0 = u(G_(a.lu.wave_base)[wave]);
    hdr.fwd_row0 = u(G_(a.solve_head_fwd.wave_base)[wave]);
    hdr.bwd_row0 = u(G_(a.solve_head_bwd.wave_base)[wave]);
    hdr.vdot_row0 = u(G_(a.vdot.wave_base)[wave]);
    hdr.jvs_row0 = u(G_(a.jvs.wave_base)[wave]);
    hdr.vdot_rows = (int)u(G_(a.vdot.rows)[wave]);
    hdr.jvs_rows = (int)u(G_(a.jvs.rows)[wave]);
  }

  double y[SPT], rct[RPT];
#pragma unroll
  for (int q = 0; q < SPT; q++) {
    const int s = q * NT + t;
    y[q] = s < NVAR ? G_(a.var_in)[(size_t)cell * NVAR + s] : 0.0;
  }
#ifndef MISTRA_RCT_RESIDENT_SLOTS
#define MISTRA_RCT_RESIDENT_SLOTS 0
#endif
  constexpr bool RCT_PER_USE = MT::WAVES_PER_SIMD > MISTRA_RESIDENT_MAX_WPS || L::RCT_IN_LDS;
  constexpr int RCT_KEEP = !RCT_PER_USE ? RPT : (MISTRA_RCT_RESIDENT_SLOTS < RPT ? MISTRA_RCT_RESIDENT_SLOTS : RPT);
  auto load_rct = [&](bool opaque) {
    const double* rc = a.rconst;
    if (opaque) asm volatile("" : "+s"(rc));
    int tt = t;
    if (opaque) asm volatile("" : "+v"(tt));
#pragma unroll
    for (int q = opaque ? RCT_KEEP : 0; q < RPT; q++) {
      const int r = q * NT + tt;
      if constexpr (L::RCT_IN_LDS) {
        if (opaque) { rct[q] = r < NREACT ? lds_ld(8u * (uint32_t)(L::RCT + r)) : 0.0; continue; }
      }
      rct[q] = r < NREACT ? G_(rc)[(size_t)cell * NREACT + r] : 0.0;
    }
  };
  if constexpr (L::RCT_IN_LDS) {
#pragma unroll
    for (int q = 0; q < RPT; q++) {
      const int r = q * NT + t;
      if (r < NREACT) lds[L::RCT + r] = G_(a.rconst)[(size_t)cell * NREACT + r];
      rct[q] = 0.0;
    }
  } else {
    load_rct(false);
  }
  constexpr bool RESIDENT = MT::WAVES_PER_SIMD <= MISTRA_RESIDENT_MAX_WPS;
  uint32_t jpos[(JPT + 1) / 2], zpos[(ZPT + 1) / 2];
  auto load_pos = [&]() {
    const uint16_t* jp = a.jvs_pos;
    const uint16_t* zp = a.zero_pos;
    int t = threadIdx.x;
    if constexpr (!RESIDENT) asm volatile("" : "+s"(jp), "+s"(zp), "+v"(t));
#pragma unroll
    for (int q = 0; q < (JPT + 1) / 2; q++)
      jpos[q] = (uint32_t)G_(jp)[(2 * q) * NT + t] | ((2 * q + 1 < JPT ? (uint32_t)G_(jp)[(2 * q + 1) * NT + t] : (uint32_t)kPosNone) << 16);
#pragma unroll
    for (int q = 0; q < (ZPT + 1) / 2; q++)
      zpos[q] = (uint32_t)G_(zp)[(2 * q) * NT + t] | ((2 * q + 1 < ZPT ? (uint32_t)G_(zp)[(2 * q + 1) * NT + t] : (uint32_t)kPosNone) << 16);
  };
  if constexpr (RESIDENT) load_pos();
#ifndef MISTRA_FFAC_RESIDENT
#define MISTRA_FFAC_RESIDENT 0
#endif
  constexpr bool FFAC_RESIDENT = RESIDENT && MISTRA_FFAC_RESIDENT;
  uint64_t ffac[RPT];
  auto load_ffac = [&]() {
    const uint64_t* ff = a.fun_fac;
    if constexpr (!FFAC_RESIDENT) asm volatile("" : "+s"(ff));
#pragma unroll
    for (int q = 0; q < RPT; q++) ffac[q] = G_(ff)[q * NT + t];
  };
  if constexpr (FFAC_RESIDENT) load_ffac();
  if (t < NFIX) X[NVAR + t] = G_(a.fix)[(size_t)cell * NFIX + t];
  if (t < NCONST) X[NVAR + NFIX + t] = G_(a.consts)[t];
  if constexpr (MT::DENSE_ND > 0) {
    if (t < 64) *(lds_u32x4*)(uintptr_t)(8u * (uint32_t)L::DINFO + 16u * (uint32_t)t) = G_(reinterpret_cast<const u32x4*>(a.dense.row_info))[t];
    for (int i = t; i < L::SCHUR_WORDS; i += NT)
      *(__attribute__((address_space(3))) uint32_t*)(uintptr_t)(8u * (uint32_t)L::SCHUR + 4u * (uint32_t)i) = G_(reinterpret_cast<const uint32_t*>(a.dense.schur_cells))[i];
  }
  if (t == 0) {
    M[NNZ + NVAR] = 0.0;
    M[NNZ + NVAR + 1] = 1.0;
    M[NNZ + NVAR + 3] = -1.0;
  }

  constexpr bool profiling = PROF;
  unsigned long long pc[kProfSlots] = {0, 0, 0, 0, 0, 0, 0, 0, 0, 0, 0, 0, 0, 0, 0, 0}, t_last = profiling ? clock64() : 0ull;
  const unsigned long long t_begin = t_last;
  auto lap = [&](int slot) {
    if constexpr (profiling) {
      const unsigned long long now = clock64();
      pc[slot] += now - t_last;
      t_last = now;
    }
  };

  bool dumping = DUMP;
  gptr_mut<double> dump = nullptr;
  if constexpr (DUMP) dump = GM_(a.dump) + (size_t)cell * (size_t)(5 * NVAR + 2 * NNZ + 2);
  auto dump_vec = [&](int at, const double (&v)[SPT]) {
    if constexpr (DUMP) {
      if (dumping) {
#pragma unroll
        for (int q = 0; q < SPT; q++) {
          const int s = q * NT + t;
          if (s < NVAR) dump[at + s] = v[q];
        }
      }
    }
  };
  auto dump_matrix = [&](int at) {
    if constexpr (DUMP) {
      if (dumping)
        for (int i = t; i < NNZ; i += NT) dump[at + i] = M[i];
    }
  };

  static_assert(SPT <= 2 && JPT * NT <= NNZ, "output cells of the gather-sum machine: at most two species per thread, JVS sums inside Ghimj");
  auto vdot_out = [&](int tt, uint32_t& addr, uint32_t& stride) {
    constexpr uint32_t trash = 8u * (uint32_t)(NNZ + NVAR + 2);
    addr = tt < NVAR ? 8u * (uint32_t)(NNZ + tt) : trash;
    if constexpr (SPT == 1) stride = tt < NVAR ? 8u * (uint32_t)NT : 0u;
    else stride = tt + NT < NVAR ? 8u * (uint32_t)NT : trash - addr;
  };
  auto fun = [&](const double (&v)[SPT], double (&out)[SPT]) {
    if constexpr (!FFAC_RESIDENT) load_ffac();
    if constexpr (RCT_PER_USE) load_rct(true);
#pragma unroll
    for (int q = 0; q < SPT; q++) {
      const int s = q * NT + t;
      if (s < NVAR) X[s] = v[q];
    }
    lds_barrier();
    {
      double f0[RPT], f1[RPT], f2[RPT];
      uint32_t slot[RPT];
#pragma unroll
      for (int q = 0; q < RPT; q++) {
        uint64_t w = ffac[q];
        asm volatile("" : "+v"(w));
        f0[q] = X[w & 0xFFFFu];
        f1[q] = X[(w >> 16) & 0xFFFFu];
        f2[q] = X[(w >> 32) & 0xFFFFu];
        slot[q] = (uint32_t)(w >> 48);
      }
#pragma unroll
      for (int q = 0; q < RPT; q++) {
        double p = rct[q] * f0[q];
        p = p * f1[q];
        p = p * f2[q];
        AB[slot[q]] = p;
      }
    }
    lds_barrier();
    lap(15);
    {
      int tt = t;
      if constexpr (!RESIDENT) asm volatile("" : "+v"(tt));
      uint32_t oa, os;
      vdot_out(tt, oa, os);
      gsum_run<NT, MT::RING_LOW>(a.vdot, hdr.vdot_row0, hdr.vdot_rows, lane, oa, os);
    }
#pragma unroll
    for (int q = 0; q < SPT; q++) {
      const int s = q * NT + t;
      out[q] = s < NVAR ? XS[s] : 0.0;
    }
  };

  double jac0[JPT];
  auto jac = [&]() {
    uint64_t jfac[3 * RPT];
    {
      const uint64_t* jf = a.jac_fac;
      asm volatile("" : "+s"(jf));
#pragma unroll
      for (int q = 0; q < 3 * RPT; q++) jfac[q] = G_(jf)[q * NT + t];
      if constexpr (RCT_PER_USE) load_rct(true);
    }
    lds_barrier();
#pragma unroll
    for (int q = 0; q < RPT; q++) {
      double f0[3], f1[3], f2[3];
#pragma unroll
      for (int b = 0; b < 3; b++) {
        const uint64_t w = jfac[q * 3 + b];
        f0[b] = X[w & 0xFFFFu];
        f1[b] = X[(w >> 16) & 0xFFFFu];
        f2[b] = X[(w >> 32) & 0xFFFFu];
      }
#pragma unroll
      for (int b = 0; b < 3; b++) {
        double p = rct[q] * f0[b];
        p = p * f1[b];
        p = p * f2[b];
        JBp[(uint32_t)(jfac[q * 3 + b] >> 48)] = p;
      }
    }
    lds_barrier();
    lap(13);
    gsum_run<NT, MT::RING_LOW>(a.jvs, hdr.jvs_row0, hdr.jvs_rows, lane, 8u * (uint32_t)t, 8u * (uint32_t)NT);
    lap(14);
#pragma unroll
    for (int q = 0; q < JPT; q++) jac0[q] = M[q * NT + t];
  };

  auto fun_jac = [&](const double (&v)[SPT], double (&out)[SPT]) {
    uint64_t jfac[3 * RPT];
    {
      const uint64_t* jf = a.jac_fac;
      asm volatile("" : "+s"(jf));
#pragma unroll
      for (int q = 0; q < 3 * RPT; q++) jfac[q] = G_(jf)[q * NT + t];
    }
    if constexpr (!FFAC_RESIDENT) load_ffac();
    if constexpr (RCT_PER_USE) load_rct(true);
#pragma unroll
    for (int q = 0; q < SPT; q++) {
      const int s = q * NT + t;
      if (s < NVAR) X[s] = v[q];
    }
    lds_barrier();
    {
      double f0[RPT], f1[RPT], f2[RPT];
      uint32_t slot[RPT];
#pragma unroll
      for (int q = 0; q < RPT; q++) {
        uint64_t w = ffac[q];
        asm volatile("" : "+v"(w));
        f0[q] = X[w & 0xFFFFu];
        f1[q] = X[(w >> 16) & 0xFFFFu];
        f2[q] = X[(w >> 32) & 0xFFFFu];
        slot[q] = (uint32_t)(w >> 48);
      }
#pragma unroll
      for (int q = 0; q < RPT; q++) {
        double p = rct[q] * f0[q];
        p = p * f1[q];
        p = p * f2[q];
        AB[slot[q]] = p;
      }
    }
#pragma unroll
    for (int q = 0; q < RPT; q++) {
      double f0[3], f1[3], f2[3];
#pragma unroll
      for (int b = 0; b < 3; b++) {
        const uint64_t w = jfac[q * 3 + b];
        f0[b] = X[w & 0xFFFFu];
        f1[b] = X[(w >> 16) & 0xFFFFu];
        f2[b] = X[(w >> 32) & 0xFFFFu];
      }
#pragma unroll
      for (int b = 0; b < 3; b++) {
        double p = rct[q] * f0[b];
        p = p * f1[b];
        p = p * f2[b];
        JBp[(uint32_t)(jfac[q * 3 + b] >> 48)] = p;
      }
    }
    lds_barrier();
    lap(13);
    {
      int tt = t;
      if constexpr (!RESIDENT) asm volatile("" : "+v"(tt));
      uint32_t oa, os;
      vdot_out(tt, oa, os);
      gsum_run<NT, MT::RING_LOW>(a.vdot, hdr.vdot_row0, hdr.vdot_rows, lane, oa, os);
    }
    gsum_run<NT, MT::RING_LOW>(a.jvs, hdr.jvs_row0, hdr.jvs_rows, lane, 8u * (uint32_t)t, 8u * (uint32_t)NT);
    lap(14);
#pragma unroll
    for (int q = 0; q < SPT; q++) {
      const int s = q * NT + t;
      out[q] = s < NVAR ? XS[s] : 0.0;
    }
#pragma unroll
    for (int q = 0; q < JPT; q++) jac0[q] = M[q * NT + t];
  };

  auto prepare = [&](double ghinv, const double (&rhs)[SPT]) -> bool {
    if constexpr (!RESIDENT) load_pos();
    if (t == 0) { flags[0] = 0; flags[1] = 0x7fffffff; }
    lds_barrier();
#pragma unroll
    for (int q = 0; q < SPT; q++) {
      const int s = q * NT + t;
      if (s < NVAR) XS[s] = rhs[q];
    }
    bool zero_diag = false;
    auto put = [&](uint32_t p, double minus_jac) {
      const bool none = p == kPosNone, dg = !none && (p & kPosDiag);
      const double vd = minus_jac + ghinv;
      const double v = dg ? vd : minus_jac;
      zero_diag |= dg && (v == 0.0);
      M[none ? (uint32_t)(NNZ + NVAR + 2) : (p & 0x7FFFu)] = v;
    };
#pragma unroll
    for (int q = 0; q < JPT; q++) {
      uint32_t pw = jpos[q / 2];
      asm volatile("" : "+v"(pw));
      put((q & 1) ? (pw >> 16) : (pw & 0xFFFFu), -jac0[q]);
    }
#pragma unroll
    for (int q = 0; q < ZPT; q++) {
      uint32_t pw = zpos[q / 2];
      asm volatile("" : "+v"(pw));
      const uint32_t p = (q & 1) ? (pw >> 16) : (pw & 0xFFFFu);
      if (q == 0) put(p, scalar_const(-0.0));
      else M[p == kPosNone ? (uint32_t)(NNZ + NVAR + 2) : (p & 0x7FFFu)] = -0.0;
    }
    if (zero_diag) flags[0] = 1;
    lds_barrier();
    return flags[0] != 0;
  };

  auto tail = [&](auto swept_tag) {
    constexpr bool SWEPT = decltype(swept_tag)::value;
    constexpr uint32_t xs_tail = 8u * (NNZ + NVAR - 64 * MT::TAIL_REGS), r_tail = 8u * (NNZ + NVAR + 4 + NVAR - 64 * MT::TAIL_REGS);
#ifndef MISTRA_LOW_BLOCK_TAIL
#define MISTRA_LOW_BLOCK_TAIL 1
#endif
    if constexpr (MT::RING_LOW && !(MISTRA_LOW_BLOCK_TAIL && MT::TAIL_REGS <= MISTRA_LOW_BLOCK_TAIL)) {
      static_assert(MT::DENSE_ND == 0, "the column form has no dense-block variant");
      tail_solve_columns<MT::TAIL_REGS, SWEPT ? MT::TAIL_REGS : 0, true>(a.tail, xs_tail, r_tail, lane);
    } else if constexpr (MT::RING_LOW) {
      tail_solve<MT::TAIL_REGS, SWEPT ? 4 * MT::TAIL_REGS : 0, true>(a.tail, xs_tail, r_tail, lane);
    } else {
      tail_solve<MT::TAIL_REGS, !SWEPT ? 0 : MT::DENSE_ND ? 4 * (MT::TAIL_REGS - 1) : 4 * MT::TAIL_REGS, false>(a.tail, xs_tail, r_tail, lane);
    }
  };
  auto solve = [&](double (&k)[SPT], bool swept) {
    for (int i = t; i < a.n_temps; i += NT) M[NNZ + 2 * NVAR + 4 + i] = 0.0;
    if (!swept) {
#pragma unroll
      for (int q = 0; q < SPT; q++) {
        const int s = q * NT + t;
        if (s < NVAR) XS[s] = k[q];
      }
      lds_barrier();
      lap(6);
      vm_run<NT, 4, kVmSweepUpdPerRec>(a.solve_head_fwd, hdr.fwd_row0, lane);
      lap(8);
      if (wave == 0)
        tail(std::false_type{});
    } else {
      lap(6);
      if (wave == 0)
        tail(std::true_type{});
    }
    lds_barrier();
    lap(9);
    vm_run<NT, 4, kVmSweepUpdPerRec>(a.solve_head_bwd, hdr.bwd_row0, lane);
    lap(10);
#pragma unroll
    for (int q = 0; q < SPT; q++) {
      const int s = q * NT + t;
      if (s < NVAR) k[q] = XS[s];
    }
  };

  auto error_norm = [&](const double (&y0)[SPT], const double (&y1)[SPT], const double (&ye)[SPT]) -> double {
    double part = 0.0;
#pragma unroll
    for (int q = 0; q < SPT; q++) {
      const int s = q * NT + t;
      if (s < NVAR) {
        const double ymax = fmax_f(fabs(y0[q]), fabs(y1[q]));
        const double scale = 1.0e-25 + 1.0e-3 * ymax;
        const double e = ye[q] / scale;
        part = part + e * e;
      }
    }
    part = wave_sum(part);
    lds_barrier();
    {
      int wv = wave;
      asm volatile("" : "+v"(wv));
      if (lane == 0) red[wv] = part;
    }
    lds_barrier();
    double sum = 0.0;
#pragma unroll
    for (int w = 0; w < NW; w++) sum += red[w];
    return sqrt(sum / (double)NVAR);
  };

  const double Tstart = a.tin, Tend = a.tout;
  const double Roundoff = 2.220446049250313e-16, Hmin = 0.0, Hmax = wave_uniform(fabs(Tend - Tstart));
  const double FacMin = 0.2, FacMax = 6.0, FacRej = 0.1, FacSafe = 0.9;
  const double Direction = (Tend >= Tstart) ? 1.0 : -1.0;
  double T = Tstart;
  const double hstart0 = (a.hstart && G_(a.hstart)[cell] > 0.0) ? G_(a.hstart)[cell] : 1.0e-3;
  auto Hget = [&]() -> double {
    int wv = wave;
    asm volatile("" : "+v"(wv));
    return wave_uniform(*(volatile lds_f64*)(uintptr_t)(8u * (uint32_t)(L::RED + L::RED_H + wv)));
  };
  auto Hset = [&](double v) {
    int wv = wave;
    asm volatile("" : "+v"(wv));
    if (lane == 0) *(volatile lds_f64*)(uintptr_t)(8u * (uint32_t)(L::RED + L::RED_H + wv)) = v;
  };
  static_assert(NW <= L::RED_H && L::RED_H + NW <= L::RED_HEXIT, "red[]: partial sums | H per wave | Hexit");
  if (t == 0) *(volatile lds_f64*)(uintptr_t)(8u * (uint32_t)(L::RED + L::RED_HEXIT)) = 0.0;
  {
    double H0 = fmin_f(fmin_f(hstart0, fabs(Tend - Tstart)), Hmax);
    if (fabs(H0) <= 10.0 * Roundoff) H0 = 1.0e-5;
    Hset(H0);
  }
  bool RejectLastH = false, RejectMoreH = false;
  int nfun = 0, njac = 0, nstp = 0, nacc = 0, nrej = 0, ndec = 0, nsol = 0, nsng = 0;
  int ierr = 1;

  double ynew[SPT], fcn0[SPT], fcn[SPT], k1[SPT], k2[SPT], k3[SPT], yerr[SPT];

  while (fabs(Tend - T) >= Roundoff) {
    if (nstp > a.max_steps) { ierr = -6; break; }
    {
      const double H = Hget();
      if (((T + scalar_const(0.1) * H) == T) || (H <= Roundoff)) { ierr = -7; break; }
      if (t == 0) *(volatile lds_f64*)(uintptr_t)(8u * (uint32_t)(L::RED + L::RED_HEXIT)) = H;
      Hset(fmin_f(H, fabs(Tend - T)));
    }

    lap(6);
    if constexpr (!RESIDENT) {
#pragma unroll
      for (int q = 0; q < JPT; q++) asm volatile("" : "=v"(jac0[q]));
    }
    if constexpr (L::MERGE_FUN_JAC) {
// ... 202 lines not shown
```

### mistra_amd/csrc/ros3_kernel.hpp

```cpp
#pragma once
#include <hip/hip_runtime.h>

#include "kernel_args.hpp"

namespace mistra {

#ifndef MISTRA_GAS_NT
#define MISTRA_GAS_NT 64
#endif
#ifndef MISTRA_AER_NT
#define MISTRA_AER_NT 256
#endif
#ifndef MISTRA_TOT_NT
#define MISTRA_TOT_NT 512
#endif
#ifndef MISTRA_GAS_WPS
#define MISTRA_GAS_WPS 3
#endif
#ifndef MISTRA_AER_WPS
#define MISTRA_AER_WPS 2
#endif
#ifndef MISTRA_AER_RING_LOW
#define MISTRA_AER_RING_LOW 0
#endif
#ifndef MISTRA_AER_SCALE_PASS
#define MISTRA_AER_SCALE_PASS 1
#endif
#ifndef MISTRA_TOT_DENSE
#define MISTRA_TOT_DENSE 1
#endif
#ifndef MISTRA_TOT_WPS
#define MISTRA_TOT_WPS 2
#endif
#ifndef MISTRA_TOT_VM_SLOTS
#define MISTRA_TOT_VM_SLOTS 4
#endif
#ifndef MISTRA_RESIDENT_MAX_WPS
#define MISTRA_RESIDENT_MAX_WPS 2
#endif
constexpr int kGasNT = MISTRA_GAS_NT, kAerNT = MISTRA_AER_NT, kTotNT = MISTRA_TOT_NT;

struct GasTraits { static constexpr int NVAR = 102, NFIX = 3, NREACT = 331, NNZ = 1110, NB = 568, NCONST = 2, NJNZ = 945, TAIL_REGS = 1, MAX_TEMPS = 10, WAVES_PER_SIMD = MISTRA_GAS_WPS, DENSE_ND = 0, DENSE_KB = 0; static constexpr bool RING_LOW = true, SCALE_PASS = false, RCT_LDS = false; static constexpr int VM_SLOTS = 4; };
struct AerTraits { static constexpr int NVAR = 257, NFIX = 5, NREACT = 979, NNZ = 6579, NB = 1598, NCONST = 2, NJNZ = 2831, TAIL_REGS = 2, MAX_TEMPS = 192, WAVES_PER_SIMD = MISTRA_AER_WPS, DENSE_ND = 0, DENSE_KB = 0; static constexpr bool RING_LOW = MISTRA_AER_RING_LOW, SCALE_PASS = MISTRA_AER_SCALE_PASS, RCT_LDS = true; static constexpr int VM_SLOTS = 4; };
struct TotTraits { static constexpr int NVAR = 417, NFIX = 7, NREACT = 1627, NNZ = 13503, NB = 2628, NCONST = 2, NJNZ = 4709, TAIL_REGS = 2, MAX_TEMPS = 768, WAVES_PER_SIMD = MISTRA_TOT_WPS, DENSE_ND = MISTRA_TOT_DENSE ? 64 : 0, DENSE_KB = MISTRA_TOT_DENSE ? 14 : 0; static constexpr bool RING_LOW = false, SCALE_PASS = true, RCT_LDS = false; static constexpr int VM_SLOTS = MISTRA_TOT_VM_SLOTS; };

constexpr int round_up2(int x) { return (x + 1) & ~1; }
constexpr int spare_cells(int nt) { return nt >= 128 ? 64 : 32; }
constexpr int max_i(int a, int b) { return a > b ? a : b; }

template <class MT, int NT>
struct LdsLayout {
  static constexpr int M = 0;
  static constexpr int X = M + round_up2(MT::NNZ + 2 * MT::NVAR + 4 + MT::MAX_TEMPS);
  static constexpr int AB = X + round_up2(MT::NVAR + MT::NFIX + MT::NCONST);
  static constexpr int AB_TRASH = max_i(MT::NREACT, MT::NB);
  static constexpr int JVS_CELLS = (MT::NJNZ + NT - 1) / NT * NT;
  static constexpr int SPARE = spare_cells(NT);
  static constexpr bool MERGE_FUN_JAC = JVS_CELLS + round_up2(AB_TRASH + SPARE) <= MT::NNZ;
  static constexpr int JB = MERGE_FUN_JAC ? M + JVS_CELLS : AB;
  static constexpr int A_CELLS = MERGE_FUN_JAC ? MT::NREACT : AB_TRASH;
  static constexpr bool RCT_IN_LDS = MERGE_FUN_JAC && MT::RCT_LDS;
  static constexpr int RCT = AB + round_up2(A_CELLS + SPARE);
  static constexpr int RED = RCT + (RCT_IN_LDS ? round_up2(MT::NREACT) : 0);
  static constexpr int RED_H = NT == 64 ? 1 : 16, RED_HEXIT = NT == 64 ? 2 : 31, RED_CELLS = NT == 64 ? 4 : 32;
  static constexpr int FLAGS = RED + RED_CELLS;
  static constexpr int DINFO = FLAGS + 2;
  static constexpr int SCHUR = DINFO + (MT::DENSE_ND > 0 ? 64 * 2 : 0);
  static constexpr int SCHUR_WORDS = MT::DENSE_ND > 0 ? 8 * MT::DENSE_KB * 64 / 2 : 0;
  static constexpr int TOTAL = SCHUR + SCHUR_WORDS / 2;
  static constexpr int PANEL = AB;
  static constexpr int PANEL_CELLS = 2 * 2 * 64 * 4 + 2 * 64 + 4;
  static_assert(MT::DENSE_ND == 0 || PANEL_CELLS <= A_CELLS + SPARE, "panel buffers must fit the product array");
  static_assert(TOTAL * 8 <= 160 * 1024, "cell state does not fit the 160 KiB LDS of a gfx950 CU");
  static_assert(NT % 64 == 0 && NT <= 1024 && NT / 64 <= 32, "workgroup size");
};

template <class MT, int NT>
hipError_t launch_ros3(const KernelArgs& a, hipStream_t stream, bool* lds_configured);

}
```

### mistra_amd/csrc/schedule.cpp

```cpp
#include "schedule.hpp"

#include <algorithm>
#include <cassert>
#include <cstdio>
#include <cstdlib>
#include <cstring>
#include <iterator>
#include <map>
#include <numeric>
#include <stdexcept>

namespace mistra {

namespace {

inline const char* diag_env(const char* name) {
#ifdef MISTRA_DIAG_ENV
  return std::getenv(name);
#else
  (void)name;
  return nullptr;
#endif
}

// ... 702 lines not shown
  const int n = m.nvar, zero_slot = lay.zero();
  T.regs = regs > 0 ? regs : n > 128 + 64 ? 2 : 1;
  T.m = 64 * T.regs;
  if (T.m > n) throw std::invalid_argument("mechanism smaller than one wave");
  T.h = n - T.m;
  if (zero_slot > 0xFFFF) throw std::invalid_argument("tail tables need 16-bit Ghimj slots");
  const uint32_t z = (uint32_t)zero_slot;
  T.fwd.assign(((size_t)T.m / 4 + VM_LOOKAHEAD_ROWS) * 256, z | (z << 16));
  T.bwd.assign(((size_t)T.m / 4 + VM_LOOKAHEAD_ROWS) * 256, z | (z << 16));
  auto put = [&](std::vector<uint32_t>& tab, int group_pos, int lane, int r, int slot) {
    uint32_t& w = tab[((size_t)(group_pos / 4) * 64 + lane) * 4 + group_pos % 4];
    w = r == 0 ? ((w & 0xFFFF0000u) | (uint32_t)slot) : ((w & 0x0000FFFFu) | ((uint32_t)slot << 16));
  };
  for (int ti = 0; ti < T.m; ti++) {
    const int i = T.h + ti, lane = ti % 64, r = ti / 64;
    for (int p = m.crow[i]; p < m.crow[i + 1]; p++) {
      const int c = m.icol[p];
      if (c < T.h || c == i) continue;
      const int q = c - T.h;
      if (c < i) put(T.fwd, q, lane, r, p);
      else put(T.bwd, T.m - 1 - q, lane, r, p);
    }
  }
  auto addresses = [](const std::vector<uint32_t>& tab, int r) {
    std::vector<uint32_t> a(tab.size());
    for (size_t k = 0; k < tab.size(); k++) a[k] = 8u * ((tab[k] >> (16 * r)) & 0xFFFFu);
    return a;
  };
  for (int r = 0; r < T.regs; r++) {
    T.fwd_addr[r] = addresses(T.fwd, r);
    T.bwd_addr[r] = addresses(T.bwd, r);
  }
  return T;
}

DenseTail build_dense_tail(const MechTables& m, const VmLayout& lay, int nd, int kb) {
  DenseTail D;
  const int n = m.nvar;
  if (nd != 64) throw std::invalid_argument("the dense tail block is 64 rows (8 waves x 2 tiles of 16x16)");
  D.nd = nd;
  D.h = n - nd;
  D.kb = kb;
  D.jm = D.h - 4 * kb;
  if (D.jm < 0 || kb < 0) throw std::invalid_argument("more Schur steps than pivots");
  if (D.info_rows() > DenseTail::kInfoRowsMax) throw std::invalid_argument("too many Schur steps for the LDS row table");
  D.row_info.assign((size_t)DenseTail::kInfoRowsMax * 4, 0u);
  auto describe_range = [&](int g, int row, int c0, int c1) {
    int first = -1, seen = 0;
    uint64_t absent = 0;
    for (int c = c0; c < c1; c++) {
      int slot = -1;
      for (int p = m.crow[row]; p < m.crow[row + 1]; p++)
        if (m.icol[p] == c) slot = p;
      if (slot < 0) { absent |= 1ull << (c - c0); continue; }
      if (first < 0) first = slot;
      if (slot != first + seen) throw std::logic_error("dense tail: a row's slots inside a column range are not contiguous");
      seen++;
    }
    for (int c = c1 - c0; c < 64; c++) absent |= 1ull << c;
    D.row_info[(size_t)g * 4] = (uint32_t)std::max(first, 0);
    D.row_info[(size_t)g * 4 + 1] = (uint32_t)absent;
    D.row_info[(size_t)g * 4 + 2] = (uint32_t)(absent >> 32);
  };
  for (int i = 0; i < nd; i++) {
    describe_range(i, D.h + i, D.h, n);
    if ((((uint64_t)D.row_info[(size_t)i * 4 + 1] | ((uint64_t)D.row_info[(size_t)i * 4 + 2] << 32)) & ~1ull) != 0)
      throw std::logic_error("dense tail: a row of the block lacks a column other than its first");
    describe_range(64 + i, D.h + i, D.jm, D.h);
  }
  for (int r = 0; r < 4 * kb; r++) describe_range(128 + r, D.jm + r, D.h, n);
  if (lay.zero() > 0xFFFF) throw std::invalid_argument("Schur cell table needs 16-bit M cells");
  D.schur_cells.assign((size_t)8 * kb * 64, (uint16_t)lay.zero());
  auto cell_or_zero = [&](int g, int c) { const int x = D.cell(g, c); return (uint16_t)(x < 0 ? lay.zero() : x); };
  for (int k = 0; k < kb; k++)
    for (int lane = 0; lane < 64; lane++) {
      const int lrow = lane >> 4, lcol = lane & 15;
      for (int I = 0; I < 4; I++) D.schur_cells[D.schur_w(I, k, lane)] = cell_or_zero(64 + 16 * I + lcol, 4 * k + lrow);
      for (int half = 0; half < 2; half++)
        for (int t = 0; t < 2; t++) D.schur_cells[D.schur_u(half, k, t, lane)] = cell_or_zero(128 + 4 * k + lrow, 16 * (2 * half + t) + lcol);
    }
  return D;
}

GsumProgram build_gsum_program(const std::vector<std::vector<std::pair<int, double>>>& outputs,
                               const std::vector<int>& slot_of_output, int nq, int nt, uint32_t src_base_bytes,
                               uint32_t zero_cell_bytes) {
  GsumProgram P;
  P.nt = nt;
  P.nw = nt / 64;
  P.nq = nq;
  std::vector<int> output_of_slot((size_t)nq * nt, -1);
  for (size_t o = 0; o < outputs.size(); o++) {
    int s = slot_of_output[o];
    if (s < 0 || s >= nq * nt || output_of_slot[(size_t)s] >= 0) throw std::logic_error("bad gsum slot map");
    output_of_slot[(size_t)s] = (int)o;
  }
  P.wave_base.assign((size_t)P.nw, 0);
  P.rows.assign((size_t)P.nw, 0);
  const float neg_zero = -0.0f;
  uint32_t neg_zero_bits;
  static_assert(sizeof neg_zero_bits == sizeof neg_zero, "float is 32 bits");
  std::memcpy(&neg_zero_bits, &neg_zero, 4);
  auto pad_row = [&]() {
    for (int l = 0; l < 64; l++) {
      for (int k = 0; k < 4; k++) P.recs.push_back(zero_cell_bytes);
      for (int k = 0; k < 4; k++) P.recs.push_back(neg_zero_bits);
    }
  };
  if (zero_cell_bytes & 7u) throw std::logic_error("gsum addresses must leave their low bits to the row marks");
  for (int w = 0; w < P.nw; w++) {
    P.wave_base[(size_t)w] = (uint32_t)(P.recs.size() / 512);
    size_t wave_rows = 0;
    for (int q = 0; q < nq; q++) {
      size_t n = 0;
      for (int l = 0; l < 64; l++) {
        int o = output_of_slot[(size_t)q * nt + w * 64 + l];
        if (o >= 0) n = std::max(n, outputs[(size_t)o].size());
      }
      const size_t rows = std::max<size_t>(1, (n + 3) / 4);
      for (size_t r = 0; r < rows; r++)
        for (int l = 0; l < 64; l++) {
          int o = output_of_slot[(size_t)q * nt + w * 64 + l];
          uint32_t addr[4], cbits[4];
          for (size_t k = 0; k < 4; k++) {
            size_t s = r * 4 + k;
            if (o >= 0 && s < outputs[(size_t)o].size()) {
              const auto& term = outputs[(size_t)o][s];
              float cf = (float)term.second;
              if ((double)cf != term.second) throw std::logic_error("stoichiometric coefficient is not a float32 value");
              if (term.first < 0 || term.first > 0xFFFF) throw std::logic_error("gsum source index out of range");
              addr[k] = src_base_bytes + 8u * (uint32_t)term.first;
              std::memcpy(&cbits[k], &cf, 4);
              P.n_terms++;
            } else {
              addr[k] = zero_cell_bytes;
              cbits[k] = neg_zero_bits;
            }
          }
          if (r == rows - 1) addr[0] |= GS_ROW_FLUSH;
          for (int k = 0; k < 4; k++) P.recs.push_back(addr[k]);
          for (int k = 0; k < 4; k++) P.recs.push_back(cbits[k]);
        }
      wave_rows += rows;
    }
    while (wave_rows % GS_ROW_ALIGN) { pad_row(); wave_rows++; }
    if (wave_rows > 0xFFFF) throw std::logic_error("gsum stream too long");
    P.rows[(size_t)w] = (uint16_t)wave_rows;
    P.wave_rows += (int64_t)wave_rows;
    for (int rr = 0; rr < VM_LOOKAHEAD_ROWS; rr++) pad_row();
  }
  return P;
}

ScaleProgram build_scale_program(const std::vector<std::pair<int, int>>& pairs, const VmLayout& lay, int nt) {
  ScaleProgram P;
  P.nt = nt;
  P.nw = nt / 64;
  P.n_pairs = (int64_t)pairs.size();
  const size_t per_lane = (pairs.size() + (size_t)nt - 1) / (size_t)nt;
  P.nslots = (int)(((per_lane + 1) / 2 + 7) / 8 * 8);
  const uint32_t trash = 8u * (uint32_t)lay.trash(), one = 8u * (uint32_t)lay.one();
  const size_t wave_slots = (size_t)P.nslots + VM_LOOKAHEAD_ROWS;
  P.recs.assign((size_t)P.nw * wave_slots * 64 * 4, 0u);
  for (size_t i = 0; i < P.recs.size(); i += 2) { P.recs[i] = trash; P.recs[i + 1] = one; }
  for (size_t i = 0; i < pairs.size(); i++) {
    const int t = (int)(i % (size_t)nt), w = t / 64, l = t % 64;
    const size_t j = i / (size_t)nt, at = (((size_t)w * wave_slots + j / 2) * 64 + (size_t)l) * 4 + 2 * (j % 2);
    P.recs[at] = 8u * (uint32_t)pairs[i].first;
    P.recs[at + 1] = 8u * (uint32_t)pairs[i].second;
  }
  return P;
}

KernelSchedule build_kernel_schedule(const MechTables& m, int nt, uint32_t ab_base_bytes, int max_temps, int dense_nd, int dense_kb,
                                     uint32_t jb_base_bytes) {
  if (nt % 64 != 0 || nt <= 0 || nt > 1024) throw std::invalid_argument("nt must be a multiple of 64 in (0,1024]");
  if (VmLayout{m.nnz, m.nvar, max_temps}.size() * 8 > 160 * 1024) throw std::invalid_argument("mechanism too large for the LDS VM");
  if (m.nx() > 0xFFFF || m.nb >= 0xFFFF || m.nreact > 0xFFFF) throw std::invalid_argument("mechanism too large");
  KernelSchedule S;
  S.nt = nt;
  S.nw = nt / 64;
  S.ab_base_bytes = ab_base_bytes;
  S.jb_base_bytes = jb_base_bytes ? jb_base_bytes : ab_base_bytes;
  const VmLayout lay{m.nnz, m.nvar, max_temps};
  const uint32_t zero_cell_bytes = 8u * (uint32_t)lay.zero();
  S.spt = ceil_div(m.nvar, nt);
  S.rpt = ceil_div(m.nreact, nt);
  const uint64_t one = (uint64_t)(m.nvar + m.nfix);

  const uint64_t ab_trash = (uint64_t)std::max(m.nreact, m.nb);
  const uint64_t a_trash = jb_base_bytes ? (uint64_t)m.nreact : ab_trash;
  const int spare = nt >= 128 ? 64 : 32;
  S.a_trash = (int)a_trash;
  S.fun_fac.resize((size_t)S.rpt * nt);
  for (size_t i = 0; i < S.fun_fac.size(); i++) S.fun_fac[i] = one | (one << 16) | (one << 32) | ((a_trash + (i % (size_t)nt) % (size_t)spare) << 48);
  for (int r = 0; r < m.nreact; r++) {
    uint64_t f[3] = {one, one, one};
    int nf = m.a_ptr[r + 1] - m.a_ptr[r];
    if (nf > 3) throw std::logic_error("reaction with more than 3 factors");
    for (int i = 0; i < nf; i++) f[i] = (uint64_t)m.a_fac[(size_t)m.a_ptr[r] + i];
    S.fun_fac[(size_t)r] = f[0] | (f[1] << 16) | (f[2] << 32) | ((uint64_t)r << 48);
  }
  {
    std::vector<std::vector<std::pair<int, double>>> outs((size_t)m.nvar);
    std::vector<int> slot((size_t)m.nvar);
    for (int s = 0; s < m.nvar; s++) {
      slot[(size_t)s] = s;
      for (int p = m.vd_ptr[s]; p < m.vd_ptr[s + 1]; p++) outs[(size_t)s].emplace_back(m.vd_idx[(size_t)p], m.vd_coef[(size_t)p]);
    }
    S.vdot = build_gsum_program(outs, slot, S.spt, nt, ab_base_bytes, zero_cell_bytes);
  }

  S.jac_fac.resize((size_t)S.rpt * 3 * nt);
  for (size_t i = 0; i < S.jac_fac.size(); i++) S.jac_fac[i] = one | (one << 16) | (one << 32) | ((ab_trash + (i % (size_t)nt) % (size_t)spare) << 48);
  {
    std::vector<int> used((size_t)m.nreact, 0);
    for (int b = 0; b < m.nb; b++) {
      int r = m.b_rct[(size_t)b];
      int k = used[(size_t)r]++;
      if (k >= 3) throw std::logic_error("more than 3 Jacobian products for one reaction");
      uint64_t f[3] = {one, one, one};
      int nf = m.b_ptr[b + 1] - m.b_ptr[b];
      if (nf > 3) throw std::logic_error("Jacobian product with more than 3 factors");
      for (int i = 0; i < nf; i++) f[i] = (uint64_t)m.b_fac[(size_t)m.b_ptr[b] + i];
      int q = r / nt, t = r % nt;
      S.jac_fac[((size_t)q * 3 + k) * nt + t] = f[0] | (f[1] << 16) | (f[2] << 32) | ((uint64_t)b << 48);
    }
  }
  {
    std::vector<int> nz, zero;
    for (int k = 0; k < m.nnz; k++) (m.jv_ptr[k + 1] > m.jv_ptr[k] ? nz : zero).push_back(k);
    S.n_jnz = (int)nz.size();
    S.n_jzero = (int)zero.size();
    S.jpt = std::max(1, ceil_div(S.n_jnz, nt));
    S.zpt = std::max(1, ceil_div(S.n_jzero, nt));
    std::vector<char> is_diag((size_t)m.nnz, 0);
    for (int s = 0; s < m.nvar; s++) is_diag[(size_t)m.diag[(size_t)s]] = 1;
    std::stable_sort(nz.begin(), nz.end(), [&](int a, int b) {
      return m.jv_ptr[a + 1] - m.jv_ptr[a] > m.jv_ptr[b + 1] - m.jv_ptr[b];
    });
    std::vector<std::vector<std::pair<int, double>>> outs(nz.size());
    std::vector<int> slot(nz.size());
    S.jvs_pos.assign((size_t)S.jpt * nt, POS_NONE);
    for (size_t i = 0; i < nz.size(); i++) {
      int k = nz[i];
      int pass = (int)(i / (size_t)nt), pos = (int)(i % (size_t)nt);
      int t = (pass & 1) ? nt - 1 - pos : pos;
      slot[i] = pass * nt + t;
      for (int p = m.jv_ptr[k]; p < m.jv_ptr[k + 1]; p++) outs[i].emplace_back(m.jv_idx[(size_t)p], m.jv_coef[(size_t)p]);
      S.jvs_pos[(size_t)slot[i]] = (uint16_t)(k | (is_diag[(size_t)k] ? POS_DIAG : 0));
    }
    S.jvs = build_gsum_program(outs, slot, S.jpt, nt, S.jb_base_bytes, zero_cell_bytes);
    S.zero_pos.assign((size_t)S.zpt * nt, POS_NONE);
    std::stable_sort(zero.begin(), zero.end(), [&](int x, int y) { return is_diag[(size_t)x] > is_diag[(size_t)y]; });
    for (size_t i = 0; i < zero.size(); i++) {
      if (is_diag[(size_t)zero[i]] && i >= (size_t)nt) throw std::logic_error("more fill-in diagonals than threads");
      S.zero_pos[i] = (uint16_t)(zero[i] | (is_diag[(size_t)zero[i]] ? POS_DIAG : 0));
    }
  }
  S.diag_pos.assign((size_t)S.spt * nt, POS_NONE);
  for (int s = 0; s < m.nvar; s++) S.diag_pos[(size_t)s] = (uint16_t)m.diag[(size_t)s];

  if (dense_nd > 0) {
    if (nt < 512) throw std::invalid_argument("the dense tail block needs eight waves");
    S.dense = build_dense_tail(m, lay, dense_nd, dense_kb);
  }
  S.tail = build_tail_solve(m, lay);
  if (dense_nd > 0 && S.tail.h > S.dense.jm) throw std::logic_error("the solves' tail chain must cover the dense block and its Schur pivots");
  const int dh = dense_nd > 0 ? S.dense.h : -1, djm = dense_nd > 0 ? S.dense.jm : -1;
  static const int local_lu = diag_env("MISTRA_DIAG_LOCAL_LU") ? std::atoi(diag_env("MISTRA_DIAG_LOCAL_LU")) : 64;
  static const int local_sweep = diag_env("MISTRA_DIAG_LOCAL_SWEEP") ? std::atoi(diag_env("MISTRA_DIAG_LOCAL_SWEEP")) : 128;
  {
    std::vector<std::pair<int, int>> pairs;
    (void)lu_entries(m, lay, true, S.tail.h, &pairs, dh, djm);
    if ((int)pairs.size() >= 16 * nt || dense_nd > 0) {
      S.lu = build_vm_program(lu_entries(m, lay, true, S.tail.h, &pairs, dh, djm), lay, nt, 2, VM_UPD_PER_REC, local_lu);
      pairs.resize(pairs.size() / 2);
      S.lu_scale = build_scale_program(pairs, lay, nt);
    } else {
      S.lu = build_vm_program(lu_entries(m, lay, true, S.tail.h, nullptr), lay, nt, 2, VM_UPD_PER_REC, local_lu);
    }
  }
  S.solve = build_vm_program(solve_entries(m, lay), lay, nt);
  {
    std::vector<VmEntry> fwd = solve_head_fwd_entries(m, lay, S.tail.h);
    static const int fwd_split = diag_env("MISTRA_DIAG_FWD_SPLIT") ? std::atoi(diag_env("MISTRA_DIAG_FWD_SPLIT")) : 6;
    S.n_temps = split_long_entries(fwd, lay, fwd_split, 0);
    static const int bwd_split = diag_env("MISTRA_DIAG_BWD_SPLIT") ? std::atoi(diag_env("MISTRA_DIAG_BWD_SPLIT")) : 4;
    int bwd_temps = 0;
    std::vector<VmEntry> bwd = solve_head_bwd_entries(m, lay, S.tail.h, bwd_split, S.n_temps, &bwd_temps);
    S.n_temps += bwd_temps;
    S.solve_head_fwd = build_vm_program(std::move(fwd), lay, nt, 2, VM_SWEEP_UPD_PER_REC, local_sweep);
    S.solve_head_bwd = build_vm_program(std::move(bwd), lay, nt, 2, VM_SWEEP_UPD_PER_REC, local_sweep);
  }
  return S;
}

std::string describe(const KernelSchedule& s) {
  char buf[2048];
  std::snprintf(buf, sizeof buf,
                "nt=%d spt=%d rpt=%d jpt=%d zpt=%d | vdot: %lld terms, %lld wave-rows | jvs: %lld terms, %lld wave-rows | "
                "LU: %d rounds, %lld updates in %lld items / %lld records, %lld wave-rows, critical %lld, %lld LDS cycles; dense tail block %d rows, %d rank-4 Schur steps | "
                "solve: tail %d rows in registers of one wave; head fwd %d rounds / %lld rows critical, head bwd %d rounds / %lld rows "
                "critical, %d partial-sum cells (whole solve as one VM program: %d rounds, %lld updates, %lld records, critical %lld)",
                s.nt, s.spt, s.rpt, s.jpt, s.zpt, (long long)s.vdot.n_terms, (long long)s.vdot.wave_rows,
                (long long)s.jvs.n_terms, (long long)s.jvs.wave_rows, s.lu.nrounds, (long long)s.lu.n_updates,
                (long long)s.lu.n_items, (long long)s.lu.n_records, (long long)s.lu.wave_rows, (long long)s.lu.crit_rows, (long long)s.lu.lds_cycles, s.dense.nd, s.dense.kb,
                s.tail.m, s.solve_head_fwd.nrounds, (long long)s.solve_head_fwd.crit_rows, s.solve_head_bwd.nrounds,
                (long long)s.solve_head_bwd.crit_rows, s.n_temps, s.solve.nrounds, (long long)s.solve.n_updates, (long long)s.solve.n_records,
                (long long)s.solve.crit_rows);
  return buf;
}

}
```

### mistra_amd/csrc/schedule.hpp

```cpp
#pragma once
#include <cstdint>
#include <string>
#include <utility>
#include <vector>

#include "kernel_args.hpp"
#include "mech_tables.hpp"

namespace mistra {

constexpr uint32_t VM_D1_RCP = 1u;
constexpr uint32_t VM_D1_CONT = 2u;
constexpr uint32_t VM_ROW_EOR = 1u << 24;
constexpr uint32_t VM_ROW_NULL = 1u << 25;
constexpr uint32_t VM_ROW_AUX = 1u << 26;
constexpr uint32_t VM_ROW_LOCAL = 1u << 27;
constexpr int VM_ROW_EOR_BIT = 24, VM_ROW_NULL_BIT = 25, VM_ROW_AUX_BIT = 26, VM_ROW_LOCAL_BIT = 27;
constexpr uint32_t VM_AUX_MASK = 0x00FFFFF8u;
constexpr int VM_REC_WORDS = 8;
inline size_t vm_rec_index(size_t row, int lane, int k) { return row * 512 + (k < 4 ? 0 : 256) + (size_t)lane * 4 + (size_t)(k & 3); }
constexpr int VM_UPD_PER_REC = 2;
constexpr int VM_SWEEP_UPD_PER_REC = kVmSweepUpdPerRec;
constexpr int VM_LOOKAHEAD_ROWS = 16;

struct VmLayout {
  int nnz = 0, nvar = 0, max_temps = 0;
  int xs(int i = 0) const { return nnz + i; }
  int zero() const { return nnz + nvar; }
  int one() const { return nnz + nvar + 1; }
  int trash() const { return nnz + nvar + 2; }
  int minus_one() const { return nnz + nvar + 3; }
  int rdiag(int k = 0) const { return nnz + nvar + 4 + k; }
  int temp(int t = 0) const { return nnz + 2 * nvar + 4 + t; }
  int size() const { return nnz + 2 * nvar + 4 + max_temps; }
};

constexpr int GS_ROW_ALIGN = 4;
constexpr uint32_t GS_ROW_FLUSH = 1u;

constexpr uint16_t POS_DIAG = 0x8000;
constexpr uint16_t POS_NONE = 0xFFFF;

struct VmUpd { int a, r, u; };

struct VmEntry {
  int tgt = 0;
  int mulr = -1;
  int rcp = -1;
  int phase = 0;
  bool keep_order = true;
  std::vector<VmUpd> upd;
};

struct VmProgram {
  int nt = 0, nw = 0, nrounds = 0, zero_slot = 0;
  int nbarriers = 0;
  int upd_per_rec = VM_UPD_PER_REC;
  std::vector<uint32_t> wave_base;
  std::vector<uint16_t> blk_n;
  std::vector<uint32_t> recs;
  int64_t n_updates = 0, n_items = 0, n_records = 0, wave_rows = 0, crit_rows = 0;
  int64_t lds_cycles = 0;
};

struct GsumProgram {
  int nt = 0, nw = 0, nq = 0;
  std::vector<uint32_t> wave_base;
  std::vector<uint16_t> rows;
  std::vector<uint32_t> recs;
  int64_t n_terms = 0, wave_rows = 0;
};

struct TailSolve {
  int m = 0, h = 0, regs = 0;
  std::vector<uint32_t> fwd;
  std::vector<uint32_t> bwd;
  std::vector<uint32_t> fwd_addr[2], bwd_addr[2];
};

struct ScaleProgram {
  int nt = 0, nw = 0, nslots = 0;
  std::vector<uint32_t> recs;
  int64_t n_pairs = 0;
};

struct DenseTail {
  int nd = 0, h = 0, jm = 0, kb = 0;
  std::vector<uint32_t> row_info;
  std::vector<uint16_t> schur_cells;
  size_t schur_w(int I, int k, int lane) const { return ((size_t)I * kb + k) * 64 + lane; }
  size_t schur_u(int half, int k, int t, int lane) const { return (size_t)4 * kb * 64 + (((size_t)half * kb + k) * 2 + t) * 64 + lane; }
  static constexpr int kInfoRowsMax = 192;
  int info_rows() const { return 128 + 4 * kb; }
  int cell(int g, int c) const {
    const uint64_t mask = (uint64_t)row_info[(size_t)g * 4 + 1] | ((uint64_t)row_info[(size_t)g * 4 + 2] << 32);
    if ((mask >> c) & 1) return -1;
    return (int)row_info[(size_t)g * 4] + c - __builtin_popcountll(mask & ((1ull << c) - 1));
  }
};

struct DenseConfig { int nd, kb; };
#ifndef MISTRA_TOT_DENSE
#define MISTRA_TOT_DENSE 1
#endif
inline DenseConfig dense_config(const MechTables& m) { return m.nvar == 417 && MISTRA_TOT_DENSE ? DenseConfig{64, 14} : DenseConfig{0, 0}; }

struct KernelSchedule {
  int nt = 0, nw = 0;
  int spt = 0;
  int rpt = 0;
  int jpt = 0;
  int zpt = 0;
  int n_jnz = 0, n_jzero = 0;
  uint32_t ab_base_bytes = 0, jb_base_bytes = 0;
  int a_trash = 0;
  std::vector<uint64_t> fun_fac;
  GsumProgram vdot;
  std::vector<uint64_t> jac_fac;
  GsumProgram jvs;
  std::vector<uint16_t> jvs_pos;
  std::vector<uint16_t> zero_pos;
  std::vector<uint16_t> diag_pos;
  VmProgram lu, solve;
  ScaleProgram lu_scale;
  VmProgram solve_head_fwd, solve_head_bwd;
  int n_temps = 0;
  TailSolve tail;
  DenseTail dense;
};

VmProgram build_vm_program(std::vector<VmEntry> entries, const VmLayout& lay, int nt, int merge_budget = 2, int upd_per_rec = VM_UPD_PER_REC,
                           int local_max = 0);
std::vector<VmEntry> lu_entries(const MechTables& m, const VmLayout& lay, bool with_rhs, int tail_h = -1,
                                std::vector<std::pair<int, int>>* scale_pairs = nullptr, int dense_h = -1, int dense_jm = -1);
DenseTail build_dense_tail(const MechTables& m, const VmLayout& lay, int nd, int kb);
ScaleProgram build_scale_program(const std::vector<std::pair<int, int>>& pairs, const VmLayout& lay, int nt);
int split_long_entries(std::vector<VmEntry>& entries, const VmLayout& lay, int threshold, int first_temp);
std::vector<VmEntry> solve_entries(const MechTables& m, const VmLayout& lay);
std::vector<VmEntry> solve_head_fwd_entries(const MechTables& m, const VmLayout& lay, int h);
std::vector<VmEntry> solve_head_bwd_entries(const MechTables& m, const VmLayout& lay, int h, int split_over = 0, int first_temp = 0,
                                            int* temps_used = nullptr);
TailSolve build_tail_solve(const MechTables& m, const VmLayout& lay, int regs = 0);
GsumProgram build_gsum_program(const std::vector<std::vector<std::pair<int, double>>>& outputs,
                               const std::vector<int>& slot_of_output, int nq, int nt, uint32_t src_base_bytes,
                               uint32_t zero_cell_bytes);
KernelSchedule build_kernel_schedule(const MechTables& m, int nt, uint32_t ab_base_bytes, int max_temps, int dense_nd = 0,
                                     int dense_kb = 0, uint32_t jb_base_bytes = 0);
std::string describe(const KernelSchedule& s);

}
```

Before: 26590 chemistry-timesteps/s.

## Split long vdot sums across lanes and fast-path one-term Jacobian outputs

For the tot mechanism, the longest species production sums are pulled out of the per-wave gather-sum program. Each lane computes weighted products and stages them into LDS strips, then chained lane groups accumulate them, so the per-wave gather rows shrink to the shorter remaining sums. Jacobian outputs in trailing passes that have only one term are computed directly as coefficient times value instead of going through the gather-sum. This adds extra LDS staging space, additional barriers and a noinline helper, and it changes summation order, which could shift rounding.

```diff
diff --git a/__graft_entry__.py b/__graft_entry__.py
--- a/__graft_entry__.py
+++ b/__graft_entry__.py
@@ -13,6 +13,7 @@
     assert os.path.exists(lib)
     subprocess.run(["make", "-s", "-C", os.path.join(REPO, "oracle")], check=True)
     subprocess.run(["make", "-s", "-C", os.path.join(REPO, "tests", "emu")], check=True)
+    subprocess.run(["make", "-s", "-C", os.path.join(REPO, "tests", "emu_long_sums")], check=True)
     if os.path.isdir("/root/reference/src") and not os.path.exists(os.path.join(REPO, "oracle", "_ref", "libmistra_ref.so")):
         subprocess.run([os.path.join(REPO, "oracle", "build_ref.sh"), "lib"], check=True)
     if os.path.isdir("/root/reference/src") and not os.path.exists(os.path.join(REPO, "oracle", "_ref", "mistra_two_pass")):
diff --git a/mistra_amd/csrc/capi.cpp b/mistra_amd/csrc/capi.cpp
--- a/mistra_amd/csrc/capi.cpp
+++ b/mistra_amd/csrc/capi.cpp
@@ -269,8 +269,9 @@
   DevBuf<double> consts;
   DevBuf<uint64_t> fun_fac, jac_fac;
   DevBuf<uint16_t> jvs_pos, zero_pos, diag_pos, schur_cells;
-  GsBufs vdot, jvs;
+  GsBufs vdot, jvs, vdot_short, jvs_short;
   VmBufs lu, solve_head_fwd, solve_head_bwd;
+  DevBuf<uint32_t> lsum_stage, lsum_dst, lsum_chain, jvs_one;
   DevBuf<uint32_t> tail_fwd, tail_bwd, tail_fwd_addr[2], tail_bwd_addr[2], lu_scale, dense_rows;
   int upload(const MechTables& t, const KernelSchedule& K) {
     n_temps = K.n_temps;
@@ -283,6 +284,14 @@
     HIP_TRY(diag_pos.upload(K.diag_pos));
     HIP_TRY(vdot.upload(K.vdot));
     HIP_TRY(jvs.upload(K.jvs));
+    if (K.long_sums) {
+      HIP_TRY(vdot_short.upload(K.vdot_short));
+      HIP_TRY(jvs_short.upload(K.jvs_short));
+      HIP_TRY(lsum_stage.upload(K.lsum.stage));
+      HIP_TRY(lsum_dst.upload(K.lsum.stage_dst));
+      HIP_TRY(lsum_chain.upload(K.lsum.chain));
+      HIP_TRY(jvs_one.upload(K.jvs_one));
+    }
     HIP_TRY(lu.upload(K.lu));
     HIP_TRY(solve_head_fwd.upload(K.solve_head_fwd));
     HIP_TRY(solve_head_bwd.upload(K.solve_head_bwd));
@@ -299,7 +308,7 @@
   }
   void release() {
     consts.release(); fun_fac.release(); jac_fac.release(); jvs_pos.release(); zero_pos.release(); diag_pos.release(); schur_cells.release();
-    vdot.release(); jvs.release(); lu.release(); solve_head_fwd.release(); solve_head_bwd.release();
+    vdot.release(); jvs.release(); vdot_short.release(); jvs_short.release(); lsum_stage.release(); lsum_dst.release(); lsum_chain.release(); jvs_one.release(); lu.release(); solve_head_fwd.release(); solve_head_bwd.release();
     tail_fwd.release(); tail_bwd.release(); lu_scale.release(); dense_rows.release();
     for (int r = 0; r < 2; r++) { tail_fwd_addr[r].release(); tail_bwd_addr[r].release(); }
   }
@@ -592,7 +601,25 @@
     const uint32_t jb_base = 8u * (uint32_t)(mech == MISTRA_MECH_GAS   ? LdsLayout<GasTraits, kGasNT>::JB
                                              : mech == MISTRA_MECH_AER ? LdsLayout<AerTraits, kAerNT>::JB
                                                                        : LdsLayout<TotTraits, kTotNT>::JB);
-    K = build_kernel_schedule(S.tab, S.nt, ab_base, max_temps, dc.nd, dc.kb, jb_base);
+    LongSumConfig ls;
+    using LT = LdsLayout<TotTraits, kTotNT>;
+    const bool long_sums = mech == MISTRA_MECH_TOT && TotTraits::LONG_SUMS;
+    if (long_sums) {
+      ls.regions = {{8u * (uint32_t)LT::LSUM, LT::LSUM_CELLS}, {8u * (uint32_t)LT::LSUM_TEMPS, LT::LSUM_TEMPS_CELLS}};
+      ls.stage_rows = TotTraits::LSUM_STAGE_ROWS;
+      ls.tau_vdot = TotTraits::LSUM_TAU;
+      ls.one_term_jvs = TotTraits::JVS_SHORT_PASSES < (TotTraits::NJNZ + kTotNT - 1) / kTotNT;
+    }
+    K = build_kernel_schedule(S.tab, S.nt, ab_base, max_temps, dc.nd, dc.kb, jb_base, long_sums ? &ls : nullptr);
+    if (long_sums) {
+      if (K.jvs_short_passes != TotTraits::JVS_SHORT_PASSES || K.lsum.stage_rows != TotTraits::LSUM_STAGE_ROWS)
+        throw std::logic_error("long sums: the schedule does not match the compiled kernel (JVS_SHORT_PASSES, LSUM_STAGE_ROWS)");
+      for (const auto& sum : K.lsum.sums) {
+        bool inside = false;
+        for (const auto& r : ls.regions) inside = inside || (sum.strip_bytes >= r.base_bytes && sum.strip_bytes + 8u * (uint32_t)sum.cells <= r.base_bytes + 8u * (uint32_t)r.cells);
+        if (!inside || sum.strip_bytes % 16u) throw std::logic_error("long sums: a strip lies outside its LDS region");
+      }
+    }
   } catch (const std::exception& ex) {
     return fail(std::string("schedule compiler: ") + ex.what());
   }
@@ -656,6 +683,9 @@
   a.consts = k.consts.p; a.fun_fac = k.fun_fac.p; a.jac_fac = k.jac_fac.p; a.jvs_pos = k.jvs_pos.p;
   a.zero_pos = k.zero_pos.p; a.diag_pos = k.diag_pos.p;
   a.vdot = k.vdot.dev(); a.jvs = k.jvs.dev(); a.lu = k.lu.dev();
+  a.vdot_short = k.vdot_short.dev(); a.jvs_short = k.jvs_short.dev();
+  a.lsum = LsDev{k.lsum_stage.p, k.lsum_dst.p, k.lsum_chain.p};
+  a.jvs_one = k.jvs_one.p;
 #ifdef MISTRA_DIAG_ENV
   if (const char* cut = std::getenv("MISTRA_DIAG_LU_ROUNDS"))
     a.lu.nrounds = std::max(1, std::min(a.lu.nrounds, std::atoi(cut)));
diff --git a/mistra_amd/csrc/kernel_args.hpp b/mistra_amd/csrc/kernel_args.hpp
--- a/mistra_amd/csrc/kernel_args.hpp
+++ b/mistra_amd/csrc/kernel_args.hpp
@@ -17,6 +17,12 @@
   const uint32_t* wave_base;
   const uint16_t* rows;
   const uint32_t* recs;
+};
+
+struct LsDev {
+  const uint32_t* stage;
+  const uint32_t* stage_dst;
+  const uint32_t* chain;
 };
 
 struct ScaleDev {
@@ -61,6 +67,9 @@
   const uint16_t* zero_pos;
   const uint16_t* diag_pos;
   GsDev vdot, jvs;
+  GsDev vdot_short, jvs_short;
+  LsDev lsum;
+  const uint32_t* jvs_one;
   VmDev lu, solve_head_fwd, solve_head_bwd;
   ScaleDev lu_scale;
   TailDev tail;
diff --git a/mistra_amd/csrc/ros3_kernel.hip b/mistra_amd/csrc/ros3_kernel.hip
--- a/mistra_amd/csrc/ros3_kernel.hip
+++ b/mistra_amd/csrc/ros3_kernel.hip
@@ -15,6 +15,7 @@
 
 typedef uint32_t u32x4 __attribute__((ext_vector_type(4)));
 typedef float f32x4 __attribute__((ext_vector_type(4)));
+typedef uint32_t u32x2 __attribute__((ext_vector_type(2)));
 
 template <class T>
 using gptr = const T __attribute__((address_space(1)))*;
@@ -717,6 +718,35 @@
 #undef MISTRA_GSUM_OPERANDS
 }
 
+typedef double f64x2 __attribute__((ext_vector_type(2)));
+typedef __attribute__((address_space(3))) f64x2 lds_f64x2;
+__device__ __forceinline__ f64x2 lds_ld2(uint32_t addr) { return *(const lds_f64x2*)(uintptr_t)addr; }
+__device__ __forceinline__ void lds_st2(uint32_t addr, double v0, double v1) { f64x2 v = {v0, v1}; *(lds_f64x2*)(uintptr_t)addr = v; }
+__device__ __forceinline__ double coef_f64(uint32_t float_bits) { return (double)__builtin_bit_cast(float, float_bits); }
+__device__ __attribute__((noinline)) uint32_t lsum_run(u32x4 a0, u32x4 c0, uint32_t d0, u32x4 a1, u32x4 c1, uint32_t d1, u32x4 chain) {
+  {
+    double x[8], p[8];
+#pragma unroll
+    for (int k = 0; k < 4; k++) { x[k] = lds_ld(a0[k]); x[4 + k] = lds_ld(a1[k]); }
+#pragma unroll
+    for (int k = 0; k < 4; k++) {
+      p[k] = coef_f64(c0[k]) * x[k];
+      p[4 + k] = coef_f64(c1[k]) * x[4 + k];
+    }
+    lds_st2(d0, p[0], p[1]); lds_st2(d0 + 16u, p[2], p[3]);
+    lds_st2(d1, p[4], p[5]); lds_st2(d1 + 16u, p[6], p[7]);
+  }
+  double acc = -0.0;
+  uint32_t at = chain.x;
+  for (uint32_t g = 0; g < chain.y; g++, at += 64u) {
+    const f64x2 v0 = lds_ld2(at), v1 = lds_ld2(at + 16u), v2 = lds_ld2(at + 32u), v3 = lds_ld2(at + 48u);
+    acc = acc + v0.x; acc = acc + v0.y; acc = acc + v1.x; acc = acc + v1.y;
+    acc = acc + v2.x; acc = acc + v2.y; acc = acc + v3.x; acc = acc + v3.y;
+  }
+  lds_st(chain.z, acc);
+  return chain.w;
+}
+
 template <int NT, bool LOW>
 __device__ __attribute__((noinline)) void scale_run(const ScaleDev P, int wave, int lane) {
   const int n = __builtin_amdgcn_readfirstlane(P.nslots);
@@ -1009,11 +1039,15 @@
     hdr.lu_row0 = u(G_(a.lu.wave_base)[wave]);
     hdr.fwd_row0 = u(G_(a.solve_head_fwd.wave_base)[wave]);
     hdr.bwd_row0 = u(G_(a.solve_head_bwd.wave_base)[wave]);
-    hdr.vdot_row0 = u(G_(a.vdot.wave_base)[wave]);
-    hdr.jvs_row0 = u(G_(a.jvs.wave_base)[wave]);
-    hdr.vdot_rows = (int)u(G_(a.vdot.rows)[wave]);
-    hdr.jvs_rows = (int)u(G_(a.jvs.rows)[wave]);
-  }
+    const GsDev& vd = MT::LONG_SUMS ? a.vdot_short : a.vdot;
+    const GsDev& jv = MT::LONG_SUMS ? a.jvs_short : a.jvs;
+    hdr.vdot_row0 = u(G_(vd.wave_base)[wave]);
+    hdr.jvs_row0 = u(G_(jv.wave_base)[wave]);
+    hdr.vdot_rows = (int)u(G_(vd.rows)[wave]);
+    hdr.jvs_rows = (int)u(G_(jv.rows)[wave]);
+  }
+  static_assert(!MT::LONG_SUMS || (LdsLayout<MT, NT>::MERGE_FUN_JAC && MT::LSUM_STAGE_ROWS == 2 && (MT::NVAR + NT - 1) / NT == 1 && MT::WAVES_PER_SIMD <= MISTRA_RESIDENT_MAX_WPS),
+                "long sums: Fun and Jac_SP in one go, two staging rows per wave, one species per thread");
 
   double y[SPT], rct[RPT];
 #pragma unroll
@@ -1129,9 +1163,25 @@
     if constexpr (SPT == 1) stride = tt < NVAR ? 8u * (uint32_t)NT : 0u;
     else stride = tt + NT < NVAR ? 8u * (uint32_t)NT : trash - addr;
   };
+  u32x4 ls_a[2], ls_c[2], ls_chain;
+  uint32_t ls_d[2];
+  auto load_lsum = [&]() {
+    const uint32_t *st = a.lsum.stage, *sd = a.lsum.stage_dst, *ch = a.lsum.chain;
+    int tt = t;
+    asm volatile("" : "+s"(st), "+s"(sd), "+s"(ch), "+v"(tt));
+    const int at = (tt >> 6) * 256 + (tt & 63);
+#pragma unroll
+    for (int r = 0; r < 2; r++) {
+      ls_a[r] = G_(reinterpret_cast<const u32x4*>(st))[at + r * 128];
+      ls_c[r] = G_(reinterpret_cast<const u32x4*>(st))[at + r * 128 + 64];
+      ls_d[r] = G_(sd)[(tt >> 6) * 128 + r * 64 + (tt & 63)];
+    }
+    ls_chain = G_(reinterpret_cast<const u32x4*>(ch))[tt];
+  };
   auto fun = [&](const double (&v)[SPT], double (&out)[SPT]) {
     if constexpr (!FFAC_RESIDENT) load_ffac();
     if constexpr (RCT_PER_USE) load_rct(true);
+    if constexpr (MT::LONG_SUMS) load_lsum();
 #pragma unroll
     for (int q = 0; q < SPT; q++) {
       const int s = q * NT + t;
@@ -1160,7 +1210,11 @@
     }
     lds_barrier();
     lap(15);
-    {
+    if constexpr (MT::LONG_SUMS) {
+      const uint32_t oa = lsum_run(ls_a[0], ls_c[0], ls_d[0], ls_a[1], ls_c[1], ls_d[1], ls_chain);
+      gsum_run<NT, MT::RING_LOW>(a.vdot_short, hdr.vdot_row0, hdr.vdot_rows, lane, oa, 0u);
+      lds_barrier();
+    } else {
       int tt = t;
       if constexpr (!RESIDENT) asm volatile("" : "+v"(tt));
       uint32_t oa, os;
@@ -1221,6 +1275,15 @@
     }
     if constexpr (!FFAC_RESIDENT) load_ffac();
     if constexpr (RCT_PER_USE) load_rct(true);
+    constexpr int JSHORT = MT::LONG_SUMS ? MT::JVS_SHORT_PASSES : JPT;
+    u32x2 jone[JPT - JSHORT + 1];
+    if constexpr (MT::LONG_SUMS) {
+      load_lsum();
+      const uint32_t* jo = a.jvs_one;
+      asm volatile("" : "+s"(jo));
+#pragma unroll
+      for (int q = JSHORT; q < JPT; q++) jone[q - JSHORT] = G_(reinterpret_cast<const u32x2*>(jo))[(q - JSHORT) * NT + t];
+    }
 #pragma unroll
     for (int q = 0; q < SPT; q++) {
       const int s = q * NT + t;
@@ -1267,14 +1330,23 @@
     }
     lds_barrier();
     lap(13);
-    {
-      int tt = t;
-      if constexpr (!RESIDENT) asm volatile("" : "+v"(tt));
-      uint32_t oa, os;
-      vdot_out(tt, oa, os);
-      gsum_run<NT, MT::RING_LOW>(a.vdot, hdr.vdot_row0, hdr.vdot_rows, lane, oa, os);
-    }
-    gsum_run<NT, MT::RING_LOW>(a.jvs, hdr.jvs_row0, hdr.jvs_rows, lane, 8u * (uint32_t)t, 8u * (uint32_t)NT);
+    if constexpr (MT::LONG_SUMS) {
+#pragma unroll
+      for (int q = JSHORT; q < JPT; q++) jac0[q] = coef_f64(jone[q - JSHORT].y) * lds_ld(jone[q - JSHORT].x);
+      const uint32_t oa = lsum_run(ls_a[0], ls_c[0], ls_d[0], ls_a[1], ls_c[1], ls_d[1], ls_chain);
+      gsum_run<NT, MT::RING_LOW>(a.vdot_short, hdr.vdot_row0, hdr.vdot_rows, lane, oa, 0u);
+      gsum_run<NT, MT::RING_LOW>(a.jvs_short, hdr.jvs_row0, hdr.jvs_rows, lane, 8u * (uint32_t)t, 8u * (uint32_t)NT);
+      lds_barrier();
+    } else {
+      {
+        int tt = t;
+        if constexpr (!RESIDENT) asm volatile("" : "+v"(tt));
+        uint32_t oa, os;
+        vdot_out(tt, oa, os);
+        gsum_run<NT, MT::RING_LOW>(a.vdot, hdr.vdot_row0, hdr.vdot_rows, lane, oa, os);
+      }
+      gsum_run<NT, MT::RING_LOW>(a.jvs, hdr.jvs_row0, hdr.jvs_rows, lane, 8u * (uint32_t)t, 8u * (uint32_t)NT);
+    }
     lap(14);
 #pragma unroll
     for (int q = 0; q < SPT; q++) {
@@ -1282,7 +1354,7 @@
       out[q] = s < NVAR ? XS[s] : 0.0;
     }
 #pragma unroll
-    for (int q = 0; q < JPT; q++) jac0[q] = M[q * NT + t];
+    for (int q = 0; q < JSHORT; q++) jac0[q] = M[q * NT + t];
   };
 
   auto prepare = [&](double ghinv, const double (&rhs)[SPT]) -> bool {
diff --git a/mistra_amd/csrc/ros3_kernel.hpp b/mistra_amd/csrc/ros3_kernel.hpp
--- a/mistra_amd/csrc/ros3_kernel.hpp
+++ b/mistra_amd/csrc/ros3_kernel.hpp
@@ -35,14 +35,24 @@
 #ifndef MISTRA_TOT_VM_SLOTS
 #define MISTRA_TOT_VM_SLOTS 4
 #endif
+#ifndef MISTRA_TOT_LONG_SUMS
+#define MISTRA_TOT_LONG_SUMS 1
+#endif
+#ifndef MISTRA_TOT_LSUM_TAU
+#define MISTRA_TOT_LSUM_TAU 0
+#endif
+#ifndef MISTRA_TOT_ONE_TERM_JVS
+#define MISTRA_TOT_ONE_TERM_JVS 1
+#endif
 #ifndef MISTRA_RESIDENT_MAX_WPS
 #define MISTRA_RESIDENT_MAX_WPS 2
 #endif
 constexpr int kGasNT = MISTRA_GAS_NT, kAerNT = MISTRA_AER_NT, kTotNT = MISTRA_TOT_NT;
 
-struct GasTraits { static constexpr int NVAR = 102, NFIX = 3, NREACT = 331, NNZ = 1110, NB = 568, NCONST = 2, NJNZ = 945, TAIL_REGS = 1, MAX_TEMPS = 10, WAVES_PER_SIMD = MISTRA_GAS_WPS, DENSE_ND = 0, DENSE_KB = 0; static constexpr bool RING_LOW = true, SCALE_PASS = false, RCT_LDS = false; static constexpr int VM_SLOTS = 4; };
-struct AerTraits { static constexpr int NVAR = 257, NFIX = 5, NREACT = 979, NNZ = 6579, NB = 1598, NCONST = 2, NJNZ = 2831, TAIL_REGS = 2, MAX_TEMPS = 192, WAVES_PER_SIMD = MISTRA_AER_WPS, DENSE_ND = 0, DENSE_KB = 0; static constexpr bool RING_LOW = MISTRA_AER_RING_LOW, SCALE_PASS = MISTRA_AER_SCALE_PASS, RCT_LDS = true; static constexpr int VM_SLOTS = 4; };
-struct TotTraits { static constexpr int NVAR = 417, NFIX = 7, NREACT = 1627, NNZ = 13503, NB = 2628, NCONST = 2, NJNZ = 4709, TAIL_REGS = 2, MAX_TEMPS = 768, WAVES_PER_SIMD = MISTRA_TOT_WPS, DENSE_ND = MISTRA_TOT_DENSE ? 64 : 0, DENSE_KB = MISTRA_TOT_DENSE ? 14 : 0; static constexpr bool RING_LOW = false, SCALE_PASS = true, RCT_LDS = false; static constexpr int VM_SLOTS = MISTRA_TOT_VM_SLOTS; };
+struct GasTraits { static constexpr int NVAR = 102, NFIX = 3, NREACT = 331, NNZ = 1110, NB = 568, NCONST = 2, NJNZ = 945, TAIL_REGS = 1, MAX_TEMPS = 10, WAVES_PER_SIMD = MISTRA_GAS_WPS, DENSE_ND = 0, DENSE_KB = 0; static constexpr bool RING_LOW = true, SCALE_PASS = false, RCT_LDS = false, LONG_SUMS = false; static constexpr int VM_SLOTS = 4, LSUM_STAGE_ROWS = 0, JVS_SHORT_PASSES = 0; };
+struct AerTraits { static constexpr int NVAR = 257, NFIX = 5, NREACT = 979, NNZ = 6579, NB = 1598, NCONST = 2, NJNZ = 2831, TAIL_REGS = 2, MAX_TEMPS = 192, WAVES_PER_SIMD = MISTRA_AER_WPS, DENSE_ND = 0, DENSE_KB = 0; static constexpr bool RING_LOW = MISTRA_AER_RING_LOW, SCALE_PASS = MISTRA_AER_SCALE_PASS, RCT_LDS = true, LONG_SUMS = false; static constexpr int VM_SLOTS = 4, LSUM_STAGE_ROWS = 0, JVS_SHORT_PASSES = 0; };
+struct TotTraits { static constexpr int NVAR = 417, NFIX = 7, NREACT = 1627, NNZ = 13503, NB = 2628, NCONST = 2, NJNZ = 4709, TAIL_REGS = 2, MAX_TEMPS = 768, WAVES_PER_SIMD = MISTRA_TOT_WPS, DENSE_ND = MISTRA_TOT_DENSE ? 64 : 0, DENSE_KB = MISTRA_TOT_DENSE ? 14 : 0; static constexpr bool RING_LOW = false, SCALE_PASS = true, RCT_LDS = false, LONG_SUMS = MISTRA_TOT_LONG_SUMS; static constexpr int VM_SLOTS = MISTRA_TOT_VM_SLOTS;
+                   static constexpr int LSUM_STAGE_ROWS = 2, JVS_SHORT_PASSES = MISTRA_TOT_ONE_TERM_JVS ? 3 : 10, LSUM_TAU = MISTRA_TOT_LSUM_TAU; };
 
 constexpr int round_up2(int x) { return (x + 1) & ~1; }
 constexpr int spare_cells(int nt) { return nt >= 128 ? 64 : 32; }
@@ -67,7 +77,12 @@
   static constexpr int DINFO = FLAGS + 2;
   static constexpr int SCHUR = DINFO + (MT::DENSE_ND > 0 ? 64 * 2 : 0);
   static constexpr int SCHUR_WORDS = MT::DENSE_ND > 0 ? 8 * MT::DENSE_KB * 64 / 2 : 0;
-  static constexpr int TOTAL = SCHUR + SCHUR_WORDS / 2;
+  static constexpr int LSUM = round_up2(SCHUR + SCHUR_WORDS / 2);
+  static constexpr int LSUM_CELLS = MT::LONG_SUMS ? 160 * 1024 / 8 - LSUM : 0;
+  static constexpr int LSUM_TEMPS = round_up2(MT::NNZ + 2 * MT::NVAR + 4);
+  static constexpr int LSUM_TEMPS_CELLS = MT::LONG_SUMS ? (MT::NNZ + 2 * MT::NVAR + 4 + MT::MAX_TEMPS - LSUM_TEMPS) / 2 * 2 : 0;
+  static_assert(!MT::LONG_SUMS || (LSUM_CELLS >= 64 && LSUM_TEMPS + LSUM_TEMPS_CELLS <= X), "long sums need staging space");
+  static constexpr int TOTAL = LSUM + LSUM_CELLS;
   static constexpr int PANEL = AB;
   static constexpr int PANEL_CELLS = 2 * 2 * 64 * 4 + 2 * 64 + 4;
   static_assert(MT::DENSE_ND == 0 || PANEL_CELLS <= A_CELLS + SPARE, "panel buffers must fit the product array");
diff --git a/mistra_amd/csrc/schedule.cpp b/mistra_amd/csrc/schedule.cpp
--- a/mistra_amd/csrc/schedule.cpp
+++ b/mistra_amd/csrc/schedule.cpp
@@ -878,6 +878,136 @@
   return P;
 }
 
+namespace {
+
+int gsum_rows_of(size_t longest) { return (int)((std::max<size_t>(1, (longest + 3) / 4) + GS_ROW_ALIGN - 1) / GS_ROW_ALIGN * GS_ROW_ALIGN); }
+
+bool try_long_sums(const std::vector<std::vector<std::pair<int, double>>>& outputs, const std::vector<uint32_t>& out_bytes, int nt,
+                   uint32_t src_base_bytes, uint32_t zero_cell_bytes, uint32_t trash_bytes, const LongSumConfig& cfg, int tau,
+                   const std::vector<int>& also_rows, LongSumProgram& P) {
+  P = LongSumProgram();
+  P.nt = nt;
+  P.nw = nt / 64;
+  P.stage_rows = cfg.stage_rows;
+  P.tau = tau;
+  const int nw = P.nw;
+  std::vector<int> order;
+  for (size_t t = 0; t < outputs.size(); t++)
+    if ((int)outputs[t].size() > tau) order.push_back((int)t);
+  std::stable_sort(order.begin(), order.end(), [&](int a, int b) { return outputs[(size_t)a].size() > outputs[(size_t)b].size(); });
+  std::vector<int> used(cfg.regions.size(), 0);
+  used[0] = 4;
+  P.dump_bytes = cfg.regions[0].base_bytes;
+  for (int t : order) {
+    const int terms = (int)outputs[(size_t)t].size(), cells = (terms + LSUM_GROUP - 1) / LSUM_GROUP * LSUM_GROUP;
+    size_t r = 0;
+    while (r < cfg.regions.size() && used[r] + cells > cfg.regions[r].cells) r++;
+    if (r == cfg.regions.size()) return false;
+    P.sums.push_back({t, -1, -1, terms, cells, cfg.regions[r].base_bytes + 8u * (uint32_t)used[r], out_bytes[(size_t)t]});
+    used[r] += cells;
+    P.n_terms += terms;
+    P.n_cells += cells;
+  }
+  std::vector<char> is_long(outputs.size(), 0);
+  for (int t : order) is_long[(size_t)t] = 1;
+  P.rows_before.assign((size_t)nw, 0);
+  P.rows_after.assign((size_t)nw, 0);
+  P.chain_groups.assign((size_t)nw, 0);
+  for (int w = 0; w < nw; w++) {
+    size_t all = 0, shrt = 0;
+    for (int l = 0; l < 64; l++) {
+      const size_t t = (size_t)w * 64 + (size_t)l;
+      if (t >= outputs.size()) break;
+      all = std::max(all, outputs[t].size());
+      if (!is_long[t]) shrt = std::max(shrt, outputs[t].size());
+    }
+    P.rows_before[(size_t)w] = gsum_rows_of(all);
+    P.rows_after[(size_t)w] = gsum_rows_of(shrt);
+  }
+  std::vector<int> count((size_t)nw, 0), pieces((size_t)nw, 0);
+  for (auto& s : P.sums) {
+    const int g = s.cells / LSUM_GROUP, np = s.cells / 4;
+    int best = -1;
+    long best_cost = 0;
+    for (int w = 0; w < nw; w++) {
+      if (count[(size_t)w] >= 64 || pieces[(size_t)w] + np > 64 * cfg.stage_rows) continue;
+      const long cost = 250L * P.rows_after[(size_t)w] + 125L * (also_rows.empty() ? 0 : also_rows[(size_t)w]) + 100L * std::max(P.chain_groups[(size_t)w], g) +
+                        4L * (pieces[(size_t)w] + np);
+      if (best < 0 || cost < best_cost) { best = w; best_cost = cost; }
+    }
+    if (best < 0) return false;
+    s.wave = best;
+    s.lane = count[(size_t)best]++;
+    pieces[(size_t)best] += np;
+    P.chain_groups[(size_t)best] = std::max(P.chain_groups[(size_t)best], g);
+  }
+  const float neg_zero = -0.0f;
+  uint32_t neg_zero_bits;
+  std::memcpy(&neg_zero_bits, &neg_zero, 4);
+  const size_t lane_rows = (size_t)nw * (size_t)cfg.stage_rows * 64;
+  P.stage.assign(lane_rows * 8, 0u);
+  P.stage_dst.assign(lane_rows, P.dump_bytes);
+  auto stage_at = [&](int w, int r, int part, int lane, int k) { return ((((size_t)w * cfg.stage_rows + r) * 2 + part) * 64 + lane) * 4 + k; };
+  for (int w = 0; w < nw; w++)
+    for (int r = 0; r < cfg.stage_rows; r++)
+      for (int l = 0; l < 64; l++)
+        for (int k = 0; k < 4; k++) {
+          P.stage[stage_at(w, r, 0, l, k)] = zero_cell_bytes;
+          P.stage[stage_at(w, r, 1, l, k)] = neg_zero_bits;
+        }
+  P.chain.assign((size_t)nt * 4, 0u);
+  for (int t = 0; t < nt; t++) {
+    P.chain[(size_t)t * 4] = P.dump_bytes;
+    P.chain[(size_t)t * 4 + 2] = trash_bytes;
+    P.chain[(size_t)t * 4 + 3] = (size_t)t < outputs.size() && !is_long[(size_t)t] ? out_bytes[(size_t)t] : trash_bytes;
+  }
+  std::fill(pieces.begin(), pieces.end(), 0);
+  for (const auto& s : P.sums) {
+    const auto& terms = outputs[(size_t)s.output];
+    for (int p = 0; p < s.cells / 4; p++) {
+      const int j = pieces[(size_t)s.wave]++, r = j / 64, l = j % 64;
+      for (int k = 0; k < 4; k++) {
+        const size_t i = (size_t)p * 4 + (size_t)k;
+        if (i >= terms.size()) continue;
+        const float cf = (float)terms[i].second;
+        if ((double)cf != terms[i].second) throw std::logic_error("stoichiometric coefficient is not a float32 value");
+        if (terms[i].first < 0 || terms[i].first > 0xFFFF) throw std::logic_error("long-sum source index out of range");
+        P.stage[stage_at(s.wave, r, 0, l, k)] = src_base_bytes + 8u * (uint32_t)terms[i].first;
+        std::memcpy(&P.stage[stage_at(s.wave, r, 1, l, k)], &cf, 4);
+      }
+      P.stage_dst[((size_t)s.wave * cfg.stage_rows + r) * 64 + l] = s.strip_bytes + 32u * (uint32_t)p;
+    }
+    const size_t t = (size_t)s.wave * 64 + (size_t)s.lane;
+    P.chain[t * 4] = s.strip_bytes;
+    P.chain[t * 4 + 1] = (uint32_t)(s.cells / LSUM_GROUP);
+    P.chain[t * 4 + 2] = s.out_bytes;
+  }
+  return true;
+}
+
+}
+
+LongSumProgram build_long_sums(const std::vector<std::vector<std::pair<int, double>>>& outputs, const std::vector<uint32_t>& out_bytes, int nt,
+                               uint32_t src_base_bytes, uint32_t zero_cell_bytes, uint32_t trash_bytes, const LongSumConfig& cfg,
+                               const std::vector<int>& also_rows) {
+  if (!also_rows.empty() && (int)also_rows.size() != nt / 64) throw std::invalid_argument("long sums: one row count per wave");
+  if (nt % 64 != 0 || (int)outputs.size() > nt || out_bytes.size() != outputs.size()) throw std::invalid_argument("long sums: one output per thread");
+  if (cfg.regions.empty() || cfg.regions[0].cells < 4 || cfg.stage_rows < 1) throw std::invalid_argument("long sums: no staging space");
+  for (const auto& r : cfg.regions)
+    if (r.base_bytes % 16u) throw std::invalid_argument("long sums: strips are read 16 bytes at a time");
+  LongSumProgram P;
+  if (cfg.tau_vdot > 0) {
+    if (!try_long_sums(outputs, out_bytes, nt, src_base_bytes, zero_cell_bytes, trash_bytes, cfg, cfg.tau_vdot, also_rows, P))
+      throw std::invalid_argument("long sums: the strips of this threshold do not fit their LDS regions or staging rows");
+    return P;
+  }
+  size_t longest = 0;
+  for (const auto& o : outputs) longest = std::max(longest, o.size());
+  for (int tau = LSUM_GROUP; tau <= (int)longest; tau += 4)
+    if (try_long_sums(outputs, out_bytes, nt, src_base_bytes, zero_cell_bytes, trash_bytes, cfg, tau, also_rows, P)) return P;
+  throw std::logic_error("long sums: no threshold fits");
+}
+
 ScaleProgram build_scale_program(const std::vector<std::pair<int, int>>& pairs, const VmLayout& lay, int nt) {
   ScaleProgram P;
   P.nt = nt;
@@ -899,7 +1029,7 @@
 }
 
 KernelSchedule build_kernel_schedule(const MechTables& m, int nt, uint32_t ab_base_bytes, int max_temps, int dense_nd, int dense_kb,
-                                     uint32_t jb_base_bytes) {
+                                     uint32_t jb_base_bytes, const LongSumConfig* long_sums) {
   if (nt % 64 != 0 || nt <= 0 || nt > 1024) throw std::invalid_argument("nt must be a multiple of 64 in (0,1024]");
   if (VmLayout{m.nnz, m.nvar, max_temps}.size() * 8 > 160 * 1024) throw std::invalid_argument("mechanism too large for the LDS VM");
   if (m.nx() > 0xFFFF || m.nb >= 0xFFFF || m.nreact > 0xFFFF) throw std::invalid_argument("mechanism too large");
@@ -918,6 +1048,7 @@
   const uint64_t a_trash = jb_base_bytes ? (uint64_t)m.nreact : ab_trash;
   const int spare = nt >= 128 ? 64 : 32;
   S.a_trash = (int)a_trash;
+  std::vector<std::vector<std::pair<int, double>>> vdot_outs;
   S.fun_fac.resize((size_t)S.rpt * nt);
   for (size_t i = 0; i < S.fun_fac.size(); i++) S.fun_fac[i] = one | (one << 16) | (one << 32) | ((a_trash + (i % (size_t)nt) % (size_t)spare) << 48);
   for (int r = 0; r < m.nreact; r++) {
@@ -935,6 +1066,7 @@
       for (int p = m.vd_ptr[s]; p < m.vd_ptr[s + 1]; p++) outs[(size_t)s].emplace_back(m.vd_idx[(size_t)p], m.vd_coef[(size_t)p]);
     }
     S.vdot = build_gsum_program(outs, slot, S.spt, nt, ab_base_bytes, zero_cell_bytes);
+    if (long_sums) vdot_outs = outs;
   }
 
   S.jac_fac.resize((size_t)S.rpt * 3 * nt);
@@ -977,12 +1109,49 @@
       S.jvs_pos[(size_t)slot[i]] = (uint16_t)(k | (is_diag[(size_t)k] ? POS_DIAG : 0));
     }
     S.jvs = build_gsum_program(outs, slot, S.jpt, nt, S.jb_base_bytes, zero_cell_bytes);
+    if (long_sums) {
+      int pshort = S.jpt;
+      while (long_sums->one_term_jvs && pshort > 0) {
+        bool one = true;
+        for (size_t i = (size_t)(pshort - 1) * nt; i < std::min(nz.size(), (size_t)pshort * nt); i++) one = one && outs[i].size() == 1;
+        if (!one) break;
+        pshort--;
+      }
+      S.jvs_short_passes = pshort;
+      const size_t nshort = std::min(nz.size(), (size_t)pshort * nt);
+      S.jvs_short = build_gsum_program(std::vector<std::vector<std::pair<int, double>>>(outs.begin(), outs.begin() + (std::ptrdiff_t)nshort),
+                                       std::vector<int>(slot.begin(), slot.begin() + (std::ptrdiff_t)nshort), std::max(1, pshort), nt, S.jb_base_bytes, zero_cell_bytes);
+      const float neg_zero = -0.0f;
+      uint32_t neg_zero_bits;
+      std::memcpy(&neg_zero_bits, &neg_zero, 4);
+      S.jvs_one.assign((size_t)(S.jpt - pshort) * nt * 2, 0u);
+      for (size_t i = 0; i < S.jvs_one.size(); i += 2) { S.jvs_one[i] = zero_cell_bytes; S.jvs_one[i + 1] = neg_zero_bits; }
+      for (size_t i = nshort; i < nz.size(); i++) {
+        const float cf = (float)outs[i][0].second;
+        if ((double)cf != outs[i][0].second) throw std::logic_error("stoichiometric coefficient is not a float32 value");
+        if (outs[i][0].first < 0 || outs[i][0].first > 0xFFFF) throw std::logic_error("gsum source index out of range");
+        const size_t at = ((size_t)slot[i] - (size_t)pshort * nt) * 2;
+        S.jvs_one[at] = S.jb_base_bytes + 8u * (uint32_t)outs[i][0].first;
+        std::memcpy(&S.jvs_one[at + 1], &cf, 4);
+      }
+    }
     S.zero_pos.assign((size_t)S.zpt * nt, POS_NONE);
     std::stable_sort(zero.begin(), zero.end(), [&](int x, int y) { return is_diag[(size_t)x] > is_diag[(size_t)y]; });
     for (size_t i = 0; i < zero.size(); i++) {
       if (is_diag[(size_t)zero[i]] && i >= (size_t)nt) throw std::logic_error("more fill-in diagonals than threads");
       S.zero_pos[i] = (uint16_t)(zero[i] | (is_diag[(size_t)zero[i]] ? POS_DIAG : 0));
     }
+  }
+  if (long_sums) {
+    if (S.spt != 1) throw std::invalid_argument("long sums: one species per thread");
+    std::vector<uint32_t> out_bytes((size_t)m.nvar);
+    std::vector<int> slot((size_t)m.nvar), jvs_rows;
+    for (int s = 0; s < m.nvar; s++) { out_bytes[(size_t)s] = 8u * (uint32_t)lay.xs(s); slot[(size_t)s] = s; }
+    for (int w = 0; w < S.nw; w++) jvs_rows.push_back(S.jvs_short.rows[(size_t)w]);
+    S.long_sums = true;
+    S.lsum = build_long_sums(vdot_outs, out_bytes, nt, ab_base_bytes, zero_cell_bytes, 8u * (uint32_t)lay.trash(), *long_sums, jvs_rows);
+    for (const auto& ls : S.lsum.sums) vdot_outs[(size_t)ls.output].clear();
+    S.vdot_short = build_gsum_program(vdot_outs, slot, S.spt, nt, ab_base_bytes, zero_cell_bytes);
   }
   S.diag_pos.assign((size_t)S.spt * nt, POS_NONE);
   for (int s = 0; s < m.nvar; s++) S.diag_pos[(size_t)s] = (uint16_t)m.diag[(size_t)s];
@@ -1035,7 +1204,24 @@
                 s.tail.m, s.solve_head_fwd.nrounds, (long long)s.solve_head_fwd.crit_rows, s.solve_head_bwd.nrounds,
                 (long long)s.solve_head_bwd.crit_rows, s.n_temps, s.solve.nrounds, (long long)s.solve.n_updates, (long long)s.solve.n_records,
                 (long long)s.solve.crit_rows);
-  return buf;
-}
-
-}
+  std::string text = buf;
+  if (s.long_sums) {
+    auto list = [](const std::vector<int>& v) {
+      std::string t;
+      for (size_t i = 0; i < v.size(); i++) t += (i ? "," : "") + std::to_string(v[i]);
+      return t;
+    };
+    std::vector<int> jb, ja;
+    for (int w = 0; w < s.nw; w++) { jb.push_back(s.jvs.rows[(size_t)w]); ja.push_back(s.jvs_short.rows[(size_t)w]); }
+    std::snprintf(buf, sizeof buf,
+                  " | long sums: vdot tau %d, %d sums, %lld terms staged into %lld strip cells by %d rows per wave; vdot rows per wave %s -> %s, "
+                  "chain groups per wave %s; jvs: %d gather-sum passes + %d one-term passes, rows per wave %s -> %s",
+                  s.lsum.tau, (int)s.lsum.sums.size(), (long long)s.lsum.n_terms, (long long)s.lsum.n_cells, s.lsum.stage_rows,
+                  list(s.lsum.rows_before).c_str(), list(s.lsum.rows_after).c_str(), list(s.lsum.chain_groups).c_str(), s.jvs_short_passes,
+                  s.jpt - s.jvs_short_passes, list(jb).c_str(), list(ja).c_str());
+    text += buf;
+  }
+  return text;
+}
+
+}
diff --git a/mistra_amd/csrc/schedule.hpp b/mistra_amd/csrc/schedule.hpp
--- a/mistra_amd/csrc/schedule.hpp
+++ b/mistra_amd/csrc/schedule.hpp
@@ -105,6 +105,26 @@
 #endif
 inline DenseConfig dense_config(const MechTables& m) { return m.nvar == 417 && MISTRA_TOT_DENSE ? DenseConfig{64, 14} : DenseConfig{0, 0}; }
 
+constexpr int LSUM_GROUP = 8;
+struct LongSumRegion { uint32_t base_bytes = 0; int cells = 0; };
+struct LongSumConfig {
+  std::vector<LongSumRegion> regions;
+  int stage_rows = 2;
+  int tau_vdot = 0;
+  bool one_term_jvs = true;
+};
+struct LongSumProgram {
+  int nt = 0, nw = 0, stage_rows = 0, tau = 0;
+  uint32_t dump_bytes = 0;
+  std::vector<uint32_t> stage;
+  std::vector<uint32_t> stage_dst;
+  std::vector<uint32_t> chain;
+  struct Sum { int output, wave, lane, terms, cells; uint32_t strip_bytes, out_bytes; };
+  std::vector<Sum> sums;
+  std::vector<int> rows_before, rows_after, chain_groups;
+  int64_t n_terms = 0, n_cells = 0;
+};
+
 struct KernelSchedule {
   int nt = 0, nw = 0;
   int spt = 0;
@@ -127,6 +147,12 @@
   int n_temps = 0;
   TailSolve tail;
   DenseTail dense;
+  bool long_sums = false;
+  LongSumProgram lsum;
+  GsumProgram vdot_short;
+  int jvs_short_passes = 0;
+  GsumProgram jvs_short;
+  std::vector<uint32_t> jvs_one;
 };
 
 VmProgram build_vm_program(std::vector<VmEntry> entries, const VmLayout& lay, int nt, int merge_budget = 2, int upd_per_rec = VM_UPD_PER_REC,
@@ -145,7 +171,10 @@
                                const std::vector<int>& slot_of_output, int nq, int nt, uint32_t src_base_bytes,
                                uint32_t zero_cell_bytes);
 KernelSchedule build_kernel_schedule(const MechTables& m, int nt, uint32_t ab_base_bytes, int max_temps, int dense_nd = 0,
-                                     int dense_kb = 0, uint32_t jb_base_bytes = 0);
+                                     int dense_kb = 0, uint32_t jb_base_bytes = 0, const LongSumConfig* long_sums = nullptr);
+LongSumProgram build_long_sums(const std::vector<std::vector<std::pair<int, double>>>& outputs, const std::vector<uint32_t>& out_bytes, int nt,
+                               uint32_t src_base_bytes, uint32_t zero_cell_bytes, uint32_t trash_bytes, const LongSumConfig& cfg,
+                               const std::vector<int>& also_rows = {});
 std::string describe(const KernelSchedule& s);
 
 }
```

Result: no change. 26800 chemistry-timesteps/s (median of 6 runs) (+0.8%).
